# SHI-Labs/SH-GAN

Hardware: AMD Instinct MI355X
Metric: generator images/sec (higher is better)
Workload: dtype f32

## Files before the change

### include/shgan_hip.h

```cpp
#ifndef SHGAN_HIP_H
#define SHGAN_HIP_H
#include <stddef.h>
#include <stdint.h>
#ifdef __cplusplus
extern "C" {
#endif

#define SHG_OK 0
#define SHG_ERR_ARG (-1)
#define SHG_ERR_LAUNCH (-2)
#define SHG_ERR_UNSUPPORTED (-3)

int shg_abi_version(void);
const char* shg_last_error(void);
int shg_device_info(int dev, char* buf, int buflen);

int shg_upfirdn2d_out_size(int H, int W, int fh, int fw, int upx, int upy, int downx, int downy, int padx0, int padx1,
                           int pady0, int pady1, int* OH, int* OW);
int shg_upfirdn2d_f32(const float* x, const float* f, float* y, int N, int C, int H, int W, int fh, int fw, int upx, int upy,
                      int downx, int downy, int padx0, int padx1, int pady0, int pady1, int flip, float gain, void* stream);
int shg_upfirdn2d_strided(const void* x, const float* f, void* y, int dtype, int N, int C, int H, int W, const long* x_strides,
                          const long* y_strides, int fh, int fw, long f_stride_y, long f_stride_x, int upx, int upy, int downx, int downy,
                          int padx0, int padx1, int pady0, int pady1, int flip, float gain, void* stream);
int shg_upfirdn2d_epilogue_f32(const float* x, const float* f, float* y, int N, int C, int H, int W, int fh, int fw, int upx,
                               int upy, int downx, int downy, int padx0, int padx1, int pady0, int pady1, int flip, float gain,
                               const float* scale, const float* bias, const float* noise, int noise_mode, float noise_strength,
                               int act, float alpha, float act_gain, float clamp, const float* residual, void* stream);

int shg_bias_act_f32(const float* x, float* y, const float* scale, const float* bias, const float* noise, int noise_mode,
                     float noise_strength, const float* residual, int N, int C, int HW, int act, float alpha, float gain,
                     float clamp, void* stream);
int shg_bias_act_backward_f32(const float* g, const float* y, float* dx, long total, int act, float alpha, float gain, float clamp,
                              void* stream);
int shg_fma_f32(const float* a, const float* b, const float* c, float* y, long total, void* stream);
int shg_fma_bcast(const void* a, const void* b, const void* c, void* y, int nd, const long* shape, const long* sa, const long* sb,
                  const long* sc, int f64, void* stream);
int shg_mul_reduce(const void* g, const void* b, void* out, int nd, int nk, const long* shape, const long* sg, const long* sb,
                   int inner_kept, int f64, void* stream);
int shg_scale_channels_f32(const float* x, const float* s, float* y, int NC, int HW, void* stream);
int shg_sum_partials_f32(const float* part, float* out, int N, int B, int K, void* stream);
int shg_scale_cast_f32_f16(const void* src, void* dst, long n, float gain, int to_half, void* stream);
int shg_planes_to_image_f32(const float* mid, const float* bias, float* y, int N, int C, int H, int W, int lo, int OH, int OW,
                            void* stream);

int shg_conv_weight_prep_f32(const float* w, float* wt, float* wscale, float* wsq, int O, int I, int KH, int KW, int OP,
                             int demod, float gain, int flip, void* stream);
int shg_conv2d_f32(const float* x, const float* wt, float* y, int NB, int I, int O, int OP, int H, int W, int kh, int kw,
                   int mode, int pad, int wgroups, long wstride, const float* in_scale, const float* out_scale,
                   const float* bias, const float* noise, int noise_mode, float noise_strength, int act, float alpha, float gain,
                   float clamp, const float* residual, int out_mode, void* workspace, size_t ws_bytes, void* stream);
size_t shg_conv2d_workspace_bytes(int NB, int I, int O, int H, int W, int kh, int kw, int mode, int pad, int wgroups);
int shg_conv_wino_chunk(void);
int shg_conv_weight_prep_wino_f32(const float* w, const float* wscale, float* wu, int O, int I, int OP, int flip, void* stream);
int shg_conv2d_wino_f32(const float* x, const float* wu, float* y, int NB, int I, int O, int OP, int H, int W,
                        const float* in_scale, const float* out_scale, const float* bias, const float* noise, int noise_mode,
                        float noise_strength, int act, float alpha, float gain, float clamp, const float* residual, void* stream);
size_t shg_conv2d_wino_workspace_bytes(int NB, int I, int O, int OP, int H, int W);
int shg_conv2d_wino_ws_f32(const float* x, const float* wu, float* y, int NB, int I, int O, int OP, int H, int W,
                           const float* in_scale, const float* out_scale, const float* bias, const float* noise, int noise_mode,
                           float noise_strength, int act, float alpha, float gain, float clamp, const float* residual, void* workspace,
                           size_t ws_bytes, void* stream);
long shg_conv_wino4_weight_elems(int OP, int I);
int shg_conv_weight_prep_wino4_f32(const float* w, const float* wscale, float* wu, int O, int I, int OP, int flip, void* stream);
int shg_conv2d_wino4_supported(int NB, int I, int O, int H, int W);
int shg_conv2d_wino4_f32(const float* x, const float* wu, float* y, int NB, int I, int O, int OP, int H, int W,
                         const float* in_scale, const float* out_scale, const float* bias, const float* noise, int noise_mode,
                         float noise_strength, int act, float alpha, float gain, float clamp, const float* residual, void* stream);
size_t shg_conv2d_wino4_workspace_bytes(int NB, int I, int O, int OP, int H, int W);
int shg_conv2d_wino4_ws_f32(const float* x, const float* wu, float* y, int NB, int I, int O, int OP, int H, int W,
                            const float* in_scale, const float* out_scale, const float* bias, const float* noise, int noise_mode,
                            float noise_strength, int act, float alpha, float gain, float clamp, const float* residual, void* workspace,
                            size_t ws_bytes, void* stream);
int shg_conv2d_wino4_route_f32(const float* x, const float* wu, float* y, int NB, int I, int O, int OP, int H, int W,
                               const float* in_scale, const float* out_scale, const float* bias, const float* noise, int noise_mode,
                               float noise_strength, int act, float alpha, float gain, float clamp, const float* residual, int route,
                               void* workspace, size_t ws_bytes, void* stream);
int shg_upfir_planar_f32(const float* mid, const float* f, float* y, int N, int C, int H, int W, int flip, float gain,
                         const float* scale, const float* bias, const float* noise, int noise_mode, float noise_strength,
                         int act, float alpha, float act_gain, float clamp, const float* residual, void* stream);
int shg_upfir_planar_sep_supported(int H, int W);
int shg_upfir_planar_sep_f32(const float* mid, const float* taps_host, float* y, int N, int C, int H, int W, int flip, float gain,
                             const float* scale, const float* bias, const float* noise, int noise_mode, float noise_strength,
                             int act, float alpha, float act_gain, float clamp, const float* residual, void* stream);
int shg_conv_weight_prep_up_poly_f32(const float* w, const float* wscale, float* wu_a, float* wu_b, int O, int I, int OP, int flip,
                                     void* stream);
int shg_conv2d_up_poly_supported(int NB, int I, int O, int H, int W);
int shg_conv2d_up_poly_f32(const float* x, const float* wt, const float* wu_a, const float* wu_b, float* y, int NB, int I, int O,
                           int OP, int H, int W, const float* in_scale, void* stream);
size_t shg_conv2d_up_poly_workspace_bytes(int NB, int I, int O, int OP, int H, int W);
int shg_conv2d_up_poly_ws_f32(const float* x, const float* wt, const float* wu_a, const float* wu_b, float* y, int NB, int I, int O,
                              int OP, int H, int W, const float* in_scale, void* workspace, size_t ws_bytes, void* stream);
int shg_fir_down_planar_f32(const float* x, const float* f, float* y, int N, int C, int H, int W, int PP, int flip, float gain,
                            void* stream);
int shg_fir_pad2_sep_supported(int H, int W, int PP);
int shg_fir_pad2_sep_f32(const float* x, const float* taps_host, float* y, int N, int C, int H, int W, int PP, int flip, float gain,
                         void* stream);
int shg_fir_resample2_sep_supported(int H, int W, int up);
int shg_fir_resample2_sep_f32(const float* x, const float* taps_host, float* y, int N, int C, int H, int W, int up, int flip, float gain,
                              void* stream);
int shg_conv_weight_prep_down_poly_f32(const float* w, const float* wscale, float* wu_a, float* wu_b, int O, int I, int OP, int flip,
                                       void* stream);
int shg_conv2d_down_poly_supported(int NB, int I, int O, int OH, int OW);
int shg_conv2d_down_poly_f32(const float* xp, const float* wu_a, const float* wu_b, float* y, int NB, int I, int O, int OP, int OH,
                             int OW, int PP, const float* in_scale, const float* bias, int act, float alpha, float gain,
                             float clamp, const float* residual, void* stream);
int shg_conv1x1_thin_in_f32(const float* x, const float* w, const float* bias, float* y, int N, int I, int O, int HW, float wgain,
                            int act, float alpha, float gain, float clamp, void* stream);
int shg_torgb_f32(const float* x, const float* w, const float* styles, const float* bias, const float* base_up, const float* f,
                  float* y, int N, int I, int O, int H, int W, void* stream);

int shg_dense_f32(const float* x, const float* w, const float* b, float* y, int N, int K, int O, int ldx, int ldy, float wgain,
                  float bgain, int act, float alpha, float gain, float clamp, void* stream);
int shg_matmul_nn_f32(const float* a, const float* b, float* out, int N, int M, int K, int lda, int ldo, float scale, void* stream);
int shg_matmul_tn_f32(const float* a, const float* b, float* out, float* colsum, int N, int M, int K, int lda, int ldb, float scale,
                      float csum_scale, void* stream);
int shg_demod_weight_f32(const float* w, float* wn, float* wsq, float* sfac, int O, int I, int K, int prenorm, void* stream);
int shg_demod_weight_backward_f32(const float* wn, const float* sfac, const float* gwn, const float* gwsq, float* gw, int O, int I, int K,
                                  void* stream);
int shg_style_factors_f32(const float* s, const float* wsq, float* sn, float* d, float* aux, int N, int I, int O, int prenorm, void* stream);
int shg_style_factors_backward_f32(const float* sn, const float* d, const float* wsq, const float* aux, const float* gsn, const float* gd,
                                   float* gs, float* gwsq, float* partq, int N, int I, int O, int prenorm, void* stream);
int shg_normalize_2nd_moment_f32(const float* x, float* y, int N, int K, float eps, void* stream);
int shg_modconv_style_prep_f32(const float* styles, int ld, const float* wsq, float* s_out, float* dcoef, int N, int I, int O,
                               int OP, int demod, float pre_gain, void* stream);

typedef struct {
    const float* x1; const float* x2; const float* w; const float* b; float* y;
    int ld1, ld2, K1, K2, O, ldy;
    float wgain, bgain;
} shg_dense_group;
int shg_dense_grouped_f32(const shg_dense_group* groups, int G, int N, void* stream);
typedef struct {
    const float* styles; const float* wsq; float* s_out; float* dcoef;
    int ld, I, O, OP, demod;
    float pre_gain;
} shg_style_group;
int shg_modconv_style_prep_grouped_f32(const shg_style_group* groups, int G, int N, void* stream);

int shg_shu_rfft2_shift_f32(const float* x, long x_batch_stride, float* T, int N, int C, void* stream);
size_t shg_conv2d_wgrad_workspace_bytes(int NB, int I, int O, int OH, int OW, int kh, int kw);
int shg_conv2d_wgrad_f32(const float* x, const float* g, float* dw, int NB, int I, int O, int H, int W, int OH, int OW,
                         int kh, int kw, int stride, int pad, void* workspace, size_t ws_bytes, void* stream);
int shg_conv2d_wgrad_wino_supported(int H, int W, int OH, int OW, int kh, int kw, int stride, int pad);
size_t shg_conv2d_wgrad_wino_workspace_bytes(int NB, int I, int O, int H, int W);
int shg_conv2d_wgrad_wino_f32(const float* x, const float* g, float* dw, int NB, int I, int O, int H, int W, void* workspace,
                              size_t ws_bytes, void* stream);
int shg_shu_spectral_f32(const float* T, const float* w0p, const float* b0, const float* w1p, const float* cw, float* S,
                         int N, int C2, int P, int bands, void* stream);
int shg_shu_split_irfft2_f32(const float* Y, const float* cw, const float* const* gauss, float* const* out,
                             const long* out_batch_stride, int N, int C, int bands, int accumulate, void* stream);
int shg_shu_split_adjoint_f32(const float* const* g, const long* g_batch_stride, const float* const* gauss, float* GS, int N, int C,
                              void* stream);
int shg_shu_rfft2_shift_n_f32(const float* x, long x_batch_stride, float* T, int N, int C, int size, void* stream);
int shg_shu_spectral_n_f32(const float* T, const float* w0p, const float* b0, const float* w1p, const float* cw, float* S,
                           int N, int C2, int P, int bands, void* stream);
int shg_shu_split_irfft2_n_f32(const float* Y, const float* cw, const float* const* gauss, float* const* out,
                               const long* out_batch_stride, int N, int C, int bands, int accumulate, int size, const int* res,
                               int levels, void* stream);
int shg_shu_split_adjoint_n_f32(const float* const* g, const long* g_batch_stride, const float* const* gauss, float* GS, int N, int C,
                                int size, const int* res, int levels, void* stream);

int shg_composite_u8(const float* x4, const float* img, uint8_t* out, int N, int H, int W, void* stream);

int shg_assemble_input_f32(const float* real, const float* mask, float* x, int N, int H, int W, void* stream);
int shg_assemble_input_u8(const uint8_t* real, const float* mask, const float* lut, float* x, int N, int H, int W, void* stream);

int shg_mask_raster_f32(const int* records, const int* offsets, const int* flips, const int* disc_table, int max_half, float* mask,
                        int* holes, int B, int s, void* stream);
int shg_mask_raster_box_f32(const int* records, const int* offsets, const int* flips, const int* disc_table, int max_half, const int* boxes,
                            float* mask, int* holes, int B, int s, void* stream);

int shg_mask_lama_f32(const int* records_host, const int* offsets_host, const int* records, const int* offsets, const int* circle_table,
                      int rmax, float* mask, int* holes, int B, int total, int s, void* stream);

// ... 104 lines not shown
```

### sh-gan_amd/_lib.py

```python
import ctypes
import os

import torch

_HERE = os.path.dirname(os.path.abspath(__file__))
LIB_PATH = os.path.join(_HERE, 'lib', 'libshgan_hip.so')
ABI_VERSION = 40

c_fp = ctypes.c_void_p
c_i = ctypes.c_int
c_f = ctypes.c_float
c_l = ctypes.c_long
c_pp = ctypes.POINTER(ctypes.c_void_p)



class DenseGroup(ctypes.Structure):
    _fields_ = [('x1', c_fp), ('x2', c_fp), ('w', c_fp), ('b', c_fp), ('y', c_fp),
                ('ld1', c_i), ('ld2', c_i), ('K1', c_i), ('K2', c_i), ('O', c_i), ('ldy', c_i),
                ('wgain', c_f), ('bgain', c_f)]


class StyleGroup(ctypes.Structure):
    _fields_ = [('styles', c_fp), ('wsq', c_fp), ('s_out', c_fp), ('dcoef', c_fp),
                ('ld', c_i), ('I', c_i), ('O', c_i), ('OP', c_i), ('demod', c_i), ('pre_gain', c_f)]


class IncConv(ctypes.Structure):
    _fields_ = [('x', c_fp), ('w', c_fp), ('bias', c_fp), ('y', c_fp)] + [
        (n, c_i) for n in ('I', 'H', 'W', 'x_ctot', 'x_coff', 'O', 'kh', 'kw', 'sh', 'sw', 'ph', 'pw', 'OH', 'OW', 'y_ctot', 'y_coff', 'splitk')]


_SIGS = {
    'shg_abi_version': [],
    'shg_device_info': [c_i, ctypes.c_char_p, c_i],
    'shg_upfirdn2d_out_size': [c_i] * 12 + [ctypes.POINTER(c_i), ctypes.POINTER(c_i)],
    'shg_upfirdn2d_f32': [c_fp, c_fp, c_fp] + [c_i] * 15 + [c_f, c_fp],
    'shg_upfirdn2d_strided': [c_fp, c_fp, c_fp, c_i, c_i, c_i, c_i, c_i, ctypes.POINTER(c_l), ctypes.POINTER(c_l), c_i, c_i, c_l, c_l] + [c_i] * 9
                             + [c_f, c_fp],
    'shg_upfirdn2d_epilogue_f32': [c_fp, c_fp, c_fp] + [c_i] * 15 + [c_f, c_fp, c_fp, c_fp, c_i, c_f, c_i, c_f, c_f, c_f, c_fp, c_fp],
    'shg_bias_act_f32': [c_fp, c_fp, c_fp, c_fp, c_fp, c_i, c_f, c_fp, c_i, c_i, c_i, c_i, c_f, c_f, c_f, c_fp],
    'shg_fma_f32': [c_fp, c_fp, c_fp, c_fp, c_l, c_fp],
    'shg_fma_bcast': [c_fp, c_fp, c_fp, c_fp, c_i] + [ctypes.POINTER(c_l)] * 4 + [c_i, c_fp],
    'shg_mul_reduce': [c_fp, c_fp, c_fp, c_i, c_i] + [ctypes.POINTER(c_l)] * 3 + [c_i, c_i, c_fp],
    'shg_scale_channels_f32': [c_fp, c_fp, c_fp, c_i, c_i, c_fp],
    'shg_sum_partials_f32': [c_fp, c_fp, c_i, c_i, c_i, c_fp],
    'shg_scale_cast_f32_f16': [c_fp, c_fp, c_l, c_f, c_i, c_fp],
    'shg_planes_to_image_f32': [c_fp, c_fp, c_fp, c_i, c_i, c_i, c_i, c_i, c_i, c_i, c_fp],
    'shg_conv_weight_prep_f32': [c_fp, c_fp, c_fp, c_fp, c_i, c_i, c_i, c_i, c_i, c_i, c_f, c_i, c_fp],
    'shg_conv2d_f32': [c_fp, c_fp, c_fp] + [c_i] * 11 + [c_l, c_fp, c_fp, c_fp, c_fp, c_i, c_f, c_i, c_f, c_f, c_f, c_fp, c_i,
                       c_fp, ctypes.c_size_t, c_fp],
    'shg_conv2d_workspace_bytes': [c_i] * 10,
    'shg_conv_wino_chunk': [],
    'shg_conv_weight_prep_wino_f32': [c_fp, c_fp, c_fp, c_i, c_i, c_i, c_i, c_fp],
    'shg_conv2d_wino_f32': [c_fp, c_fp, c_fp] + [c_i] * 6 + [c_fp, c_fp, c_fp, c_fp, c_i, c_f, c_i, c_f, c_f, c_f, c_fp, c_fp],
    'shg_conv2d_wino_ws_f32': [c_fp, c_fp, c_fp] + [c_i] * 6 + [c_fp, c_fp, c_fp, c_fp, c_i, c_f, c_i, c_f, c_f, c_f, c_fp, c_fp, ctypes.c_size_t, c_fp],
    'shg_conv2d_wino_workspace_bytes': [c_i] * 6,
    'shg_conv_wino4_weight_elems': [c_i, c_i],
    'shg_conv_weight_prep_wino4_f32': [c_fp, c_fp, c_fp, c_i, c_i, c_i, c_i, c_fp],
    'shg_conv2d_wino4_supported': [c_i] * 5,
    'shg_conv2d_wino4_f32': [c_fp, c_fp, c_fp] + [c_i] * 6 + [c_fp, c_fp, c_fp, c_fp, c_i, c_f, c_i, c_f, c_f, c_f, c_fp, c_fp],
    'shg_conv2d_wino4_ws_f32': [c_fp, c_fp, c_fp] + [c_i] * 6 + [c_fp, c_fp, c_fp, c_fp, c_i, c_f, c_i, c_f, c_f, c_f, c_fp, c_fp, ctypes.c_size_t, c_fp],
    'shg_conv2d_wino4_route_f32': [c_fp, c_fp, c_fp] + [c_i] * 6 + [c_fp, c_fp, c_fp, c_fp, c_i, c_f, c_i, c_f, c_f, c_f, c_fp, c_i, c_fp, ctypes.c_size_t, c_fp],
    'shg_conv2d_wino4_workspace_bytes': [c_i] * 6,
    'shg_upfir_planar_f32': [c_fp, c_fp, c_fp, c_i, c_i, c_i, c_i, c_i, c_f, c_fp, c_fp, c_fp, c_i, c_f, c_i, c_f, c_f, c_f, c_fp, c_fp],
    'shg_upfir_planar_sep_supported': [c_i, c_i],
    'shg_upfir_planar_sep_f32': [c_fp, ctypes.POINTER(c_f), c_fp, c_i, c_i, c_i, c_i, c_i, c_f, c_fp, c_fp, c_fp, c_i, c_f, c_i, c_f, c_f, c_f, c_fp, c_fp],
    'shg_conv1x1_thin_in_f32': [c_fp, c_fp, c_fp, c_fp, c_i, c_i, c_i, c_i, c_f, c_i, c_f, c_f, c_f, c_fp],
    'shg_torgb_f32': [c_fp, c_fp, c_fp, c_fp, c_fp, c_fp, c_fp, c_i, c_i, c_i, c_i, c_i, c_fp],
    'shg_dense_f32': [c_fp, c_fp, c_fp, c_fp, c_i, c_i, c_i, c_i, c_i, c_f, c_f, c_i, c_f, c_f, c_f, c_fp],
    'shg_demod_weight_f32': [c_fp, c_fp, c_fp, c_fp, c_i, c_i, c_i, c_i, c_fp],
    'shg_demod_weight_backward_f32': [c_fp, c_fp, c_fp, c_fp, c_fp, c_i, c_i, c_i, c_fp],
    'shg_style_factors_f32': [c_fp, c_fp, c_fp, c_fp, c_fp, c_i, c_i, c_i, c_i, c_fp],
    'shg_style_factors_backward_f32': [c_fp, c_fp, c_fp, c_fp, c_fp, c_fp, c_fp, c_fp, c_fp, c_i, c_i, c_i, c_i, c_fp],
    'shg_matmul_nn_f32': [c_fp, c_fp, c_fp, c_i, c_i, c_i, c_i, c_i, c_f, c_fp],
    'shg_matmul_tn_f32': [c_fp, c_fp, c_fp, c_fp, c_i, c_i, c_i, c_i, c_i, c_f, c_f, c_fp],
    'shg_normalize_2nd_moment_f32': [c_fp, c_fp, c_i, c_i, c_f, c_fp],
    'shg_modconv_style_prep_f32': [c_fp, c_i, c_fp, c_fp, c_fp, c_i, c_i, c_i, c_i, c_i, c_f, c_fp],
    'shg_dense_grouped_f32': [ctypes.POINTER(DenseGroup), c_i, c_i, c_fp],
    'shg_modconv_style_prep_grouped_f32': [ctypes.POINTER(StyleGroup), c_i, c_i, c_fp],
    'shg_shu_rfft2_shift_f32': [c_fp, c_l, c_fp, c_i, c_i, c_fp],
    'shg_bias_act_backward_f32': [c_fp, c_fp, c_fp, c_l, c_i, c_f, c_f, c_f, c_fp],
    'shg_conv2d_wgrad_workspace_bytes': [c_i] * 7,
    'shg_conv2d_wgrad_f32': [c_fp, c_fp, c_fp] + [c_i] * 11 + [c_fp, ctypes.c_size_t, c_fp],
    'shg_conv2d_wgrad_wino_supported': [c_i] * 8,
    'shg_conv2d_wgrad_wino_workspace_bytes': [c_i] * 5,
    'shg_conv2d_wgrad_wino_f32': [c_fp, c_fp, c_fp] + [c_i] * 5 + [c_fp, ctypes.c_size_t, c_fp],
    'shg_shu_spectral_f32': [c_fp] * 6 + [c_i] * 4 + [c_fp],
    'shg_shu_split_irfft2_f32': [c_fp, c_fp, c_pp, c_pp, ctypes.POINTER(c_l), c_i, c_i, c_i, c_i, c_fp],
    'shg_shu_split_adjoint_f32': [c_pp, ctypes.POINTER(c_l), c_pp, c_fp, c_i, c_i, c_fp],
    'shg_shu_rfft2_shift_n_f32': [c_fp, c_l, c_fp, c_i, c_i, c_i, c_fp],
    'shg_shu_spectral_n_f32': [c_fp] * 6 + [c_i] * 4 + [c_fp],
    'shg_shu_split_irfft2_n_f32': [c_fp, c_fp, c_pp, c_pp, ctypes.POINTER(c_l), c_i, c_i, c_i, c_i, c_i, ctypes.POINTER(c_i), c_i, c_fp],
    'shg_shu_split_adjoint_n_f32': [c_pp, ctypes.POINTER(c_l), c_pp, c_fp, c_i, c_i, c_i, ctypes.POINTER(c_i), c_i, c_fp],
    'shg_composite_u8': [c_fp, c_fp, c_fp, c_i, c_i, c_i, c_fp],
    'shg_assemble_input_f32': [c_fp, c_fp, c_fp, c_i, c_i, c_i, c_fp],
    'shg_assemble_input_u8': [c_fp, c_fp, c_fp, c_fp, c_i, c_i, c_i, c_fp],
    'shg_conv_weight_prep_up_poly_f32': [c_fp, c_fp, c_fp, c_fp, c_i, c_i, c_i, c_i, c_fp],
    'shg_conv2d_up_poly_supported': [c_i, c_i, c_i, c_i, c_i],
    'shg_conv2d_up_poly_f32': [c_fp, c_fp, c_fp, c_fp, c_fp, c_i, c_i, c_i, c_i, c_i, c_i, c_fp, c_fp],
    'shg_conv2d_up_poly_ws_f32': [c_fp, c_fp, c_fp, c_fp, c_fp] + [c_i] * 6 + [c_fp, c_fp, ctypes.c_size_t, c_fp],
    'shg_conv2d_up_poly_workspace_bytes': [c_i] * 6,
    'shg_fir_down_planar_f32': [c_fp, c_fp, c_fp, c_i, c_i, c_i, c_i, c_i, c_i, c_f, c_fp],
    'shg_fir_pad2_sep_supported': [c_i, c_i, c_i],
    'shg_fir_resample2_sep_supported': [c_i, c_i, c_i],
    'shg_fir_resample2_sep_f32': [c_fp, ctypes.POINTER(c_f), c_fp, c_i, c_i, c_i, c_i, c_i, c_i, c_f, c_fp],
    'shg_fir_pad2_sep_f32': [c_fp, ctypes.POINTER(c_f), c_fp, c_i, c_i, c_i, c_i, c_i, c_i, c_f, c_fp],
    'shg_conv_weight_prep_down_poly_f32': [c_fp, c_fp, c_fp, c_fp, c_i, c_i, c_i, c_i, c_fp],
    'shg_conv2d_down_poly_supported': [c_i, c_i, c_i, c_i, c_i],
    'shg_conv2d_down_poly_f32': [c_fp, c_fp, c_fp, c_fp, c_i, c_i, c_i, c_i, c_i, c_i, c_i, c_fp, c_fp, c_i, c_f, c_f, c_f, c_fp, c_fp],
    'shg_mask_raster_f32': [c_fp, c_fp, c_fp, c_fp, c_i, c_fp, c_fp, c_i, c_i, c_fp],
    'shg_mask_raster_box_f32': [c_fp, c_fp, c_fp, c_fp, c_i, c_fp, c_fp, c_fp, c_i, c_i, c_fp],
    'shg_mask_lama_f32': [c_fp, c_fp, c_fp, c_fp, c_fp, c_i, c_fp, c_fp, c_i, c_i, c_i, c_fp],
    'shg_fid_accumulate_f64': [c_fp, c_i, c_fp, c_fp, c_i, c_i, c_i, c_fp],
    'shg_inception_frontend_f32': [c_fp, c_fp, c_f, c_f, c_fp, c_i, c_i, c_i, c_fp],
    'shg_inception_packed_weight_elems': [c_i] * 4,
    'shg_inception_weight_prep_f32': [c_fp, c_fp, c_fp, c_fp, c_i, c_i, c_i, c_i, c_fp],
    'shg_inception_conv_workspace_bytes': [ctypes.POINTER(IncConv), c_i, c_i],
    'shg_inception_conv_f32': [ctypes.POINTER(IncConv), c_i, c_i, c_fp, ctypes.c_size_t, c_fp],
    'shg_inception_pool_f32': [c_fp, c_fp] + [c_i] * 9 + [c_fp],
    'shg_inception_mean_f32': [c_fp, c_fp, c_i, c_i, c_i, c_fp],
    'shg_inception_head_f32': [c_fp, c_fp, c_fp, c_fp, c_i, c_i, c_i, c_fp],
    'shg_kid_workspace_bytes': [c_i, c_i],
    'shg_kid_sums_f64': [c_fp, c_fp, c_i, c_i, c_i, c_i, c_fp, c_fp, c_i, c_i, c_fp, ctypes.c_size_t, c_fp, c_fp],
    'shg_is_accumulate_f64': [c_fp, c_fp, c_fp, c_i, c_i, c_i, c_fp],
    'shg_pr_workspace_bytes': [c_i, c_i, c_i],
    'shg_pr_radii_f16': [c_fp, c_i, c_i, c_i, c_fp, ctypes.c_size_t, c_fp, c_fp],
    'shg_pr_inside_f16': [c_fp, c_i, c_fp, c_i, c_i, c_fp, c_fp, ctypes.c_size_t, c_fp, c_fp],
    'shg_vgg16_frontend_f32': [c_fp, c_fp, c_f, c_f, ctypes.POINTER(c_f), ctypes.POINTER(c_f), c_fp, c_i, c_i, c_i, c_fp],
    'shg_vgg16_maxpool2_f32': [c_fp, c_fp, c_i, c_i, c_i, c_i, c_fp],
    'shg_lpips_conv1_weight_prep_f32': [c_fp, c_fp, c_fp, c_fp, c_fp],
    'shg_lpips_conv1_f32': [c_fp, c_fp, c_f, c_f, ctypes.POINTER(c_f), ctypes.POINTER(c_f), c_fp, c_fp, c_fp, c_i, c_i, c_i, c_fp],
    'shg_lpips_head_scratch_bytes': [c_i] * 3,
    'shg_lpips_head_f32': [c_fp, c_fp, c_fp, c_i, c_i, c_i, c_i, c_fp, ctypes.c_size_t, c_fp, c_fp],
    'shg_lpips_scaling_f32': [c_fp, c_fp, c_f, c_f, ctypes.POINTER(c_f), ctypes.POINTER(c_f), c_fp, c_i, c_i, c_i, c_fp],
    'shg_ppl_frontend_f32': [c_fp, c_fp, c_i, c_i, c_i, c_i, c_i, c_i, ctypes.POINTER(c_f), ctypes.POINTER(c_f), c_fp],
    'shg_adam_tick': [c_fp, c_i, c_fp, c_i, c_fp, c_fp, c_fp],
    'shg_adam_buckets_f32': [c_fp, c_i, c_l, c_fp, c_f, c_i, c_i, c_fp],
    'shg_ema_lerp_f32': [c_fp, c_i, c_l, c_fp, c_fp],
    'shg_image_metrics_scratch_bytes': [c_i] * 4,
    'shg_image_metrics': [c_fp, c_fp, c_f, c_f, c_fp, c_fp, c_f, c_f] + [c_i] * 6 + [c_fp, ctypes.c_size_t, c_fp, c_fp, c_fp],
    'shg_resize_bicubic_u8': [c_fp, c_l, c_fp, c_l, c_fp, c_i, c_i, c_i, c_i, c_i, c_fp],
    'shg_resize_fit_pad_u8': [c_fp, c_l, c_fp, c_l, c_fp, c_i, c_i, c_i, c_i, c_i, c_fp],
    'shg_randcrop_bicubic_ragged_f32': [c_fp, c_l, ctypes.POINTER(c_i), c_fp, c_fp, c_fp, c_i, c_i, c_fp],
    'shg_randcrop_bicubic_planar_f32': [c_fp, c_l, ctypes.POINTER(c_i), c_fp, c_fp, c_fp, c_i, c_i, c_fp],
    'shg_minibatch_std_f32': [c_fp, c_fp, c_fp, c_i, c_i, c_i, c_i, c_i, c_i, c_fp],
    'shg_conv2d_f16': [c_fp, c_fp, c_fp, c_fp] + [c_i] * 12 + [c_fp],
    'shg_conv2d_f16_needs_clear': [c_i] * 5,
    'shg_conv2d_f16_fused': [c_fp, c_fp, c_fp] + [c_i] * 12 + [c_fp, c_fp, c_fp, c_i, c_f, c_fp, c_i, c_f, c_f, c_f, c_fp, c_fp],
    'shg_conv2d_f16_packed_weight_elems': [c_i] * 3,
    'shg_conv2d_f16_pack_weight': [c_fp, c_fp, c_i, c_i, c_i, c_fp],
    'shg_conv2d_f16_pack_weight_oihw': [c_fp, c_fp, c_i, c_i, c_i, c_i, c_i, c_fp],
    'shg_conv2d_f16_set_routes': [c_i],
    'shg_conv2d_wgrad_f16_workspace_bytes': [c_i] * 6,
    'shg_conv2d_wgrad_f16': [c_fp, c_fp, c_fp] + [c_i] * 10 + [c_fp, ctypes.c_size_t, c_fp],
    'shg_upfirdn2d_f16': [c_fp, c_fp, c_fp] + [c_i] * 15 + [c_f, c_fp],
    'shg_relayout_f32_f16': [c_fp, c_fp, c_i, c_i, c_l, c_i, c_fp],
    'shg_bias_act_f16': [c_fp, c_fp, c_fp, c_l, c_i, c_i, c_f, c_f, c_f, c_fp],
    'shg_bias_act_backward_f16': [c_fp, c_fp, c_fp, c_l, c_i, c_f, c_f, c_f, c_fp],
    'shg_modtail_backward_f32_blocks': [c_l],
    'shg_modtail_backward_f32_cslices': [c_i, c_i, c_l],
    'shg_modtail_backward_f32': [c_fp] * 9 + [c_i, c_i, c_l, c_i, c_f, c_f, c_f, c_fp],
    'shg_modtail_f16': [c_fp, c_fp, c_fp, c_i, c_fp, c_fp, c_i, c_l, c_i, c_i, c_f, c_f, c_f, c_fp],
    'shg_modtail_backward_f16_blocks': [c_l, c_i],
    'shg_modtail_backward_f16': [c_fp] * 9 + [c_i, c_l, c_i, c_i, c_f, c_f, c_f, c_fp],
}

_lib = None


class ShgError(RuntimeError):
    """Raised when a C-ABI call returns a negative status (mirrors TORCH_CHECK -> RuntimeError)."""


def get_lib():
    global _lib
    if _lib is not None:
        return _lib
    if not os.path.exists(LIB_PATH):
        raise RuntimeError(
            f'{LIB_PATH} not found: the HIP extension is not built. Run `python sh-gan_amd/build.py` '
            '(or __graft_entry__.build()). There is deliberately no CPU / PyTorch fallback.')
    lib = ctypes.CDLL(LIB_PATH)
    for name, args in _SIGS.items():
        fn = getattr(lib, name)
        fn.argtypes = args
        fn.restype = c_i
    lib.shg_last_error.argtypes = []
    lib.shg_last_error.restype = ctypes.c_char_p
    lib.shg_conv2d_workspace_bytes.restype = ctypes.c_size_t
    lib.shg_conv2d_wgrad_workspace_bytes.restype = ctypes.c_size_t
    lib.shg_conv2d_wino_workspace_bytes.restype = ctypes.c_size_t
    lib.shg_conv2d_wino4_workspace_bytes.restype = ctypes.c_size_t
    lib.shg_conv2d_up_poly_workspace_bytes.restype = ctypes.c_size_t
    lib.shg_conv2d_wgrad_wino_workspace_bytes.restype = ctypes.c_size_t
    lib.shg_conv2d_wgrad_f16_workspace_bytes.restype = ctypes.c_size_t
    lib.shg_image_metrics_scratch_bytes.restype = ctypes.c_size_t
    lib.shg_lpips_head_scratch_bytes.restype = ctypes.c_size_t
    lib.shg_inception_conv_workspace_bytes.restype = ctypes.c_size_t
    lib.shg_kid_workspace_bytes.restype = ctypes.c_size_t
    lib.shg_pr_workspace_bytes.restype = ctypes.c_size_t
    lib.shg_inception_packed_weight_elems.restype = c_l
    lib.shg_conv2d_f16_packed_weight_elems.restype = c_l
    lib.shg_conv_wino4_weight_elems.restype = c_l
    ver = lib.shg_abi_version()
    if ver != ABI_VERSION:
        raise RuntimeError(f'libshgan_hip.so ABI {ver} != expected {ABI_VERSION}: rebuild with sh-gan_amd/build.py')
    _lib = lib
    return lib


def exported_symbols():
    return sorted(list(_SIGS.keys()) + ['shg_last_error'])


def check(rc, what=''):
    if rc != 0:
        msg = get_lib().shg_last_error().decode(errors='replace')
        raise ShgError(f'{what}: {msg} (code {rc})')
```

### sh-gan_amd/csrc/conv_wino_poly.hip

```cpp
#include "wino_common.h"
#include <stdlib.h>
#include <type_traits>

__device__ __attribute__((aligned(16))) float shg_poly_zeros[64];

struct PolySub {
    const float* wu;
    int nby, nbx;
    int tiles_x, tiles_y;
    int n_ttiles;
};
struct PolyParams {
    const float* x;
    float* y;
    const float* in_scale;
    int NB, I, O, OP, H, W;
    int n_otiles, nchunk;
    PolySub a, b;
    const float* wt;
    int IPK, n_strip_tiles;
    int PH2, PP;
    const float* bias;
    const float* residual;
    int act;
    float alpha, gain, clamp;
    int cps;
    long part_stride;
};

namespace poly {
constexpr int KC = 8, BO = 64, BT = 64;
constexpr int V_SZ = 16 * KC * BT;
constexpr int NT = 1024;
constexpr int NXF = KC;

enum { UA = 0, UB = 1, DA = 2, DB = 3 };

template <int SCHEME, int TY, int TX, int NBX>
struct Geo {
    static constexpr bool A = SCHEME == UA || SCHEME == DA;
    static_assert(NBX > 0 || TY * TX == BT, "64 blocks per tile");
    static_assert(NBX == 0 || A, "flat tiling is for the 3x3 blocks of schemes UA / DA");
    static constexpr int BS = A ? 3 : 2;
    static constexpr int RMAX = NBX ? (NBX - 1 + BT + NBX - 1) / NBX : TY;
    static constexpr int PH = A ? 3 * RMAX + 1 : 2 * TY + 1;
    static constexpr int PW = SCHEME == UA ? ((3 * (NBX ? NBX : TX) + 1 + 3 + 3) / 4) * 4
                            : SCHEME == DA ? (NBX ? ((3 * NBX + 1 + 3) / 4) * 4 : ((3 * TX + 1 + 3 + 3) / 4) * 4)
                            : 2 * TX + 4;
    static constexpr int DB_W0 = 2 * TX, DB_W1 = 2 * TX + 4, DB_W2 = 2 * TX;
    static constexpr int DB_N0 = (2 * TY + 1) * DB_W0, DB_N1 = 2 * TY * DB_W1, DB_N2 = 2 * TY * DB_W2;
    static constexpr int RP = SCHEME == DB ? DB_N0 + DB_N1 + DB_N2 : PH * PW;
    static constexpr int PW4 = PW / 4, PATCH4 = RP / 4, R_SZ = KC * RP;
    static constexpr int NPIECE = (PATCH4 + 63) / 64;
};
}

template <int SCHEME, int TY, int TX, int NBX>
__device__ __forceinline__ void poly_body(const PolyParams& p, const PolySub& q, const int bid, float* __restrict__ Vl,
                                          float* __restrict__ Rl) {
    using namespace poly;
    using G = Geo<SCHEME, TY, TX, NBX>;
    constexpr int PW = G::PW, PW4 = G::PW4, PATCH4 = G::PATCH4, RP = G::RP, R_SZ = G::R_SZ, BS = G::BS, NPIECE = G::NPIECE;
    constexpr bool FLAT = NBX > 0;
    constexpr bool DOWN = SCHEME == DA || SCHEME == DB;
    const int c0 = DOWN ? 0 : blockIdx.y * p.cps, nch = DOWN ? p.nchunk : min(p.cps, p.nchunk - c0), iend = min(p.I, (c0 + nch) * poly::KC);

    const int tid = threadIdx.x;
    const int lane = tid & 63, wave = __builtin_amdgcn_readfirstlane(tid >> 6);
    const int l31 = lane & 31, half = lane >> 5;

    const int nwork = q.n_ttiles * p.n_otiles;
    const int work = shg_xcd_remap(bid, nwork);
    const int otile = work / q.n_ttiles;
    const int ttile = work - otile * q.n_ttiles;
    const int txb = ttile % q.tiles_x;
    const int tyb = (ttile / q.tiles_x) % q.tiles_y;
    const int n = ttile / (q.tiles_x * q.tiles_y);
    const int id0 = txb * BT;
    const int by0 = FLAT ? id0 / (NBX ? NBX : 1) : tyb * TY, bx0 = FLAT ? 0 : txb * TX;
    const int o0 = otile * BO;
    const int HW = DOWN ? p.PH2 * p.PP : p.H * p.W;
    const int wy0 = DOWN ? BS * by0 : BS * by0 - 1;
    const int wx0 = SCHEME == UA ? ((3 * bx0 - 1) & ~3) : SCHEME == DA ? ((3 * bx0) & ~3) : SCHEME == UB ? 2 * bx0 - 4 : 2 * bx0;
    const int coff = (DOWN ? BS * bx0 : BS * bx0 - 1) - wx0;

    const bool xformer = wave < NXF;
    constexpr int NLD = 16 - NXF;
    constexpr int CPL = (KC + NLD - 1) / NLD;
    int roff[NPIECE];
#pragma unroll
    for (int j = 0; j < NPIECE; ++j) {
        const int e = j * 64 + lane;
        if constexpr (SCHEME == DB) {
            constexpr int N0 = G::DB_N0 / 4, N1 = G::DB_N1 / 4, W0 = G::DB_W0 / 4, W1 = G::DB_W1 / 4, W2 = G::DB_W2 / 4;
            const int pl = e < N0 ? 1 : (e < N0 + N1 ? 2 : 3);
            const int r4 = e < N0 ? e : (e < N0 + N1 ? e - N0 : e - N0 - N1);
            const int w4 = pl == 1 ? W0 : (pl == 2 ? W1 : W2);
            const int py = r4 / w4, p4 = r4 - py * w4;
            const int iy = wy0 + py, ix = wx0 + 4 * p4;
            const bool ok = e < PATCH4 && iy < p.PH2 && ix + 3 < p.PP;
            roff[j] = ok ? (pl * p.NB + n) * p.I * HW + iy * p.PP + ix : -1;
        } else {
            const int py = e / PW4, p4 = e - py * PW4;
            const int iy = wy0 + py, ix = wx0 + 4 * p4;
            if constexpr (SCHEME == DA) {
                const bool ok = e < PATCH4 && iy < p.PH2 && ix + 3 < p.PP;
                roff[j] = ok ? n * p.I * HW + iy * p.PP + ix : -1;
            } else {
                const bool ok = e < PATCH4 && iy >= 0 && iy < p.H && ix >= 0 && ix + 3 < p.W;
                roff[j] = ok ? n * p.I * HW + iy * p.W + ix : -1;
// ... 89 lines not shown
            for (int cc = 1; cc < 3; ++cc) {
                vb[(0 * 2 + cc - 1) * KC * BT] = d[0][cc] - d[1][cc];
                vb[(1 * 2 + cc - 1) * KC * BT] = d[1][cc];
                vb[(2 * 2 + cc - 1) * KC * BT] = d[2][cc] - d[1][cc];
            }
#pragma unroll
            for (int r = 1; r < 3; ++r) {
                vb[(6 + (r - 1) * 3 + 0) * KC * BT] = d[r][0] - d[r][1];
                vb[(6 + (r - 1) * 3 + 1) * KC * BT] = d[r][1];
                vb[(6 + (r - 1) * 3 + 2) * KC * BT] = d[r][2] - d[r][1];
            }
#pragma unroll
            for (int r = 1; r < 3; ++r)
#pragma unroll
                for (int cc = 1; cc < 3; ++cc) vb[(12 + (r - 1) * 2 + cc - 1) * KC * BT] = d[r][cc];
        }
    };

    f32x16 acc[2][2];
#pragma unroll
    for (int ob = 0; ob < 2; ++ob)
#pragma unroll
        for (int tb = 0; tb < 2; ++tb)
#pragma unroll
            for (int r = 0; r < 16; ++r) acc[ob][tb][r] = 0.f;
    const float* bbase = Vl + (wave * KC + half) * BT + l31;

    load_u(ua, 0);
    if (!xformer) {
        dma_raw(0, 0);
        if (nch > 1) dma_raw(1, 1);
    }
    asm volatile("s_waitcnt vmcnt(0)" ::: "memory");
    __syncthreads();
    if (xformer) transform(0, 0);
    __syncthreads();

    float b[2][2], apend[2];
    auto mma = [&](float a0, float a1, int buf) __attribute__((always_inline)) {
#pragma unroll
        for (int tb = 0; tb < 2; ++tb) acc[0][tb] = __builtin_amdgcn_mfma_f32_32x32x2f32(a0, b[buf][tb], acc[0][tb], 0, 0, 0);
#pragma unroll
        for (int tb = 0; tb < 2; ++tb) acc[1][tb] = __builtin_amdgcn_mfma_f32_32x32x2f32(a1, b[buf][tb], acc[1][tb], 0, 0, 0);
    };
    auto chunk = [&](auto par, int c) __attribute__((always_inline)) {
        constexpr int PAR = decltype(par)::value;
        f32x4 (&ucur)[NU] = PAR ? ub : ua;
        f32x4 (&unxt)[NU] = PAR ? ua : ub;
        const bool more = c + 1 < nch;
        const float* bb = bbase + PAR * V_SZ;
        auto fetch = [&](int ks, int buf) __attribute__((always_inline)) {
#pragma unroll
            for (int tb = 0; tb < 2; ++tb) b[buf][tb] = bb[(ks * 2) * BT + tb * 32];
        };
        fetch(0, 0);
        __builtin_amdgcn_sched_barrier(0);
        if (c > 0) mma(apend[0], apend[1], 1);
        __builtin_amdgcn_sched_barrier(0);
        if (more) load_u(unxt, c + 1);
        if (!xformer) {
            if (c + 2 < nch) dma_raw(c + 2, PAR);
        } else if (more) {
            transform(c + 1, PAR ^ 1);
        }
        __builtin_amdgcn_sched_barrier(0);
#pragma unroll
        for (int ks = 0; ks < KC / 2 - 1; ++ks) {
            fetch(ks + 1, (ks + 1) & 1);
            __builtin_amdgcn_sched_barrier(0);
            mma(ucur[(ks * 2) / 4][(ks * 2) % 4], ucur[(ks * 2 + 1) / 4][(ks * 2 + 1) % 4], ks & 1);
        }
        apend[0] = ucur[(KC - 2) / 4][(KC - 2) % 4];
        apend[1] = ucur[(KC - 1) / 4][(KC - 1) % 4];
        asm volatile("s_waitcnt lgkmcnt(0)" ::: "memory");
        __syncthreads();
    };
    for (int c = 0; c < nch; c += 2) {
        chunk(std::integral_constant<int, 0>{}, c);
        if (c + 1 < nch) chunk(std::integral_constant<int, 1>{}, c + 1);
    }
    mma(apend[0], apend[1], 1);

    float* Mx = Vl;
    const int PWg = DOWN ? p.W : p.W + 1;
    const long plane = DOWN ? (long)p.H * p.W : (long)(p.H + 1) * PWg;
    const int o_l = tid >> 5, t_l = tid & 31;
    f32x2 pre_part[SCHEME == DB ? 4 : 1][2], pre_res[SCHEME == DB ? 4 : 1][2];
    float pre_bias[2] = {0.f, 0.f};
    const ShgAct actc = shg_act_make(p.act, p.alpha, p.gain, p.clamp);
    if constexpr (SCHEME == DB) {
#pragma unroll
        for (int pass = 0; pass < 4; ++pass) {
            const int ob = pass >> 1, t = (pass & 1) * 32 + t_l;
            const int by = by0 + t / TX, bx = bx0 + t % TX;
            const int o = min(o0 + ob * 32 + o_l, p.O - 1);
            if ((pass & 1) == 0) pre_bias[ob] = p.bias ? p.bias[o] : 0.f;
#pragma unroll
            for (int j = 0; j < 2; ++j) {
                pre_part[pass][j] = f32x2{0.f, 0.f};
                pre_res[pass][j] = f32x2{0.f, 0.f};
                if (by < q.nby && bx < q.nbx && 2 * by + j < p.H) {
                    const long off = ((long)n * p.O + o) * plane + (long)(2 * by + j) * PWg + 2 * bx;
                    pre_part[pass][j] = *reinterpret_cast<const f32x2*>(p.y + off);
                    if (p.residual) pre_res[pass][j] = *reinterpret_cast<const f32x2*>(p.residual + off);
                }
            }
        }
    }
#pragma unroll
    for (int pass = 0; pass < 4; ++pass) {
        const int ob = pass >> 1, tb = pass & 1;
#pragma unroll
        for (int r = 0; r < 16; ++r) {
            const int row = (r & 3) + 8 * (r >> 2) + 4 * half;
            Mx[(wave * 32 + row) * 32 + l31] = acc[ob][tb][r];
        }
        __syncthreads();
        float m[16];
#pragma unroll
        for (int xi = 0; xi < 16; ++xi) m[xi] = Mx[(xi * 32 + o_l) * 32 + t_l];
        const int t = tb * 32 + t_l;
        const int by = FLAT ? (id0 + t) / (NBX ? NBX : 1) : by0 + t / TX, bx = FLAT ? (id0 + t) % (NBX ? NBX : 1) : bx0 + t % TX;
        const int o = o0 + ob * 32 + o_l;
        if (o < p.O && by < q.nby && bx < q.nbx) {
            float* yb = p.y + (DOWN ? 0 : blockIdx.y * p.part_stride) + ((long)n * p.O + o) * plane;
            const long pstride = (long)p.NB * p.O * plane;
            if constexpr (G::A) {
                float t3[3][4];
#pragma unroll
                for (int cc = 0; cc < 4; ++cc) {
                    t3[0][cc] = m[0 * 4 + cc] + m[1 * 4 + cc] + m[2 * 4 + cc];
                    t3[1][cc] = m[1 * 4 + cc] - m[2 * 4 + cc];
                    t3[2][cc] = m[1 * 4 + cc] + m[2 * 4 + cc] - m[3 * 4 + cc];
                }
                constexpr int EXT = DOWN ? 0 : 1;
#pragma unroll
                for (int i = 0; i < 3; ++i) {
                    const int u = 3 * by + i;
                    if (u >= p.H + EXT) continue;
                    const float y0 = t3[i][0] + t3[i][1] + t3[i][2], y1 = t3[i][1] - t3[i][2], y2 = t3[i][1] + t3[i][2] - t3[i][3];
                    float* yr = yb + (long)u * PWg + 3 * bx;
                    yr[0] = y0;
                    if (3 * bx + 1 < p.W + EXT) yr[1] = y1;
                    if (3 * bx + 2 < p.W + EXT) yr[2] = y2;
                }
            } else if constexpr (SCHEME == DB) {
                const int p0 = 2 * by, q0 = 2 * bx;
                const float bs = pre_bias[ob];
#pragma unroll
                for (int j = 0; j < 2; ++j) {
                    if (p0 + j >= p.H) continue;
                    float* yr = yb + (long)(p0 + j) * PWg + q0;
                    const f32x2 part = pre_part[pass][j];
                    const f32x2 rs = pre_res[pass][j];
                    f32x2 out;
#pragma unroll
                    for (int cc = 0; cc < 2; ++cc) {
                        float v = part[cc] + m[j * 2 + cc] + m[(j + 1) * 2 + cc]
                                + m[6 + j * 3 + cc] + m[6 + j * 3 + cc + 1]
                                + m[12 + j * 2 + cc] + bs;
                        out[cc] = shg_act_apply(v, actc) + rs[cc];
                    }
                    *reinterpret_cast<f32x2*>(yr) = out;
                }
            } else {
                const int u0 = 2 * by, v0 = 2 * bx;
                float* yeo = yb + pstride + (long)u0 * PWg + v0;
                float* yoe = yb + 2 * pstride + (long)u0 * PWg + v0;
                float* yoo = yb + 3 * pstride + (long)u0 * PWg + v0;
#pragma unroll
                for (int cc = 0; cc < 2; ++cc) {
                    yeo[cc] = m[0 * 2 + cc] + m[1 * 2 + cc];
                    yeo[PWg + cc] = m[1 * 2 + cc] + m[2 * 2 + cc];
                }
#pragma unroll
                for (int r = 0; r < 2; ++r) {
                    yoe[r * PWg] = m[6 + r * 3] + m[6 + r * 3 + 1];
                    yoe[r * PWg + 1] = m[6 + r * 3 + 1] + m[6 + r * 3 + 2];
                    yoo[r * PWg] = m[12 + r * 2];
                    yoo[r * PWg + 1] = m[12 + r * 2 + 1];
                }
            }
        }
        if (pass < 3) __syncthreads();
    }
}

__device__ __forceinline__ void poly_strip_body(const PolyParams& p, const int tile, const int wave, float* __restrict__ redbuf) {
    float (*red)[16][64] = reinterpret_cast<float (*)[16][64]>(redbuf);
    const float* wt = p.wt;
    const int IPK = p.IPK;
    const int lane = threadIdx.x & 63;
    const int l31 = lane & 31, half = lane >> 5;
    const int nseg_r = (p.W + 31) / 32, nseg_c = (p.H + 31) / 32;
    const int no32 = p.OP / 32;
    const bool live = tile < p.n_strip_tiles;
    int seg = tile % (nseg_r + nseg_c);
    const int ot32 = (tile / (nseg_r + nseg_c)) % no32;
    const int n = live ? tile / ((nseg_r + nseg_c) * no32) : 0;
    const bool col = seg >= nseg_r;
    if (col) seg -= nseg_r;
    const int len = col ? p.H : p.W;
    const int pos = seg * 32 + l31;
    const int tap = col ? 1 * 3 + 2 : 2 * 3 + 1;
    const int HW = p.H * p.W;
    const bool pok = live && pos < len;
    const float* xb = p.x + (long)n * p.I * HW + (pok ? (col ? pos * p.W + p.W - 1 : (p.H - 1) * p.W + pos) : 0);
    const float* wb = wt + ((long)(ot32 >> 1) * IPK + tap) * 64 + (ot32 & 1) * 32 + l31;
    const float* sb = p.in_scale ? p.in_scale + (long)n * p.I : nullptr;
    const int i_lo = blockIdx.y * p.cps * poly::KC, i_hi = min(p.I, i_lo + p.cps * poly::KC);
    const int kper = ((i_hi - i_lo + 7) / 8) * 2;
    const int kbeg = i_lo + wave * kper, kend = min(i_hi, kbeg + kper);
    f32x16 acc;
#pragma unroll
    for (int r = 0; r < 16; ++r) acc[r] = 0.f;
    for (int i0 = kbeg; i0 < kend; i0 += 32) {
        float a[16], bv[16];
#pragma unroll
        for (int k = 0; k < 16; ++k) {
            const int ic = i0 + 2 * k + half;
            const int i = min(ic, p.I - 1);
            a[k] = wb[(long)i * 9 * 64];
            bv[k] = xb[(long)i * HW];
            if (sb) bv[k] *= sb[i];
            if (ic >= kend) a[k] = 0.f;
            if (ic >= kend || !pok) bv[k] = 0.f;
        }
#pragma unroll
        for (int k = 0; k < 16; ++k) acc = __builtin_amdgcn_mfma_f32_32x32x2f32(a[k], bv[k], acc, 0, 0, 0);
    }
#pragma unroll
    for (int r = 0; r < 16; ++r) red[wave][r][lane] = acc[r];
    __syncthreads();
    if (!pok) return;
    const int PWg = p.W + 1;
    const long plane = (long)(p.H + 1) * PWg;
    const long pix = col ? (long)pos * PWg + p.W : (long)p.H * PWg + pos;
    float* yb = p.y + blockIdx.y * p.part_stride + (long)(col ? 2 : 1) * p.NB * p.O * plane + (long)n * p.O * plane + pix;
#pragma unroll
    for (int rr = 0; rr < 4; ++rr) {
        const int r = wave * 4 + rr;
        const float v = red[0][r][lane] + red[1][r][lane] + red[2][r][lane] + red[3][r][lane];
        const int o = ot32 * 32 + (r & 3) + 8 * (r >> 2) + 4 * half;
        if (o < p.O) yb[(long)o * plane] = v;
    }
}

template <int ATY, int ATX, int ANBX, int BTY, int BTX>
__global__ __launch_bounds__(1024) void conv_poly_up_kernel(const PolyParams p) {
    using namespace poly;
    using GA = Geo<UA, ATY, ATX, ANBX>;
    using GB = Geo<UB, BTY, BTX, 0>;
    constexpr int R_MAX = GA::R_SZ > GB::R_SZ ? GA::R_SZ : GB::R_SZ;
    __shared__ __attribute__((aligned(16))) float Vl[2 * V_SZ];
    __shared__ __attribute__((aligned(16))) float Rl[2 * R_MAX];
    const int nA = p.a.n_ttiles * p.n_otiles, nB = p.b.n_ttiles * p.n_otiles;
    if ((int)blockIdx.x < nA) poly_body<UA, ATY, ATX, ANBX>(p, p.a, blockIdx.x, Vl, Rl);
    else if ((int)blockIdx.x < nA + nB) poly_body<UB, BTY, BTX, 0>(p, p.b, blockIdx.x - nA, Vl, Rl);
    else {
        const int wave = threadIdx.x >> 6;
        poly_strip_body(p, (blockIdx.x - nA - nB) * 4 + (wave >> 2), wave & 3, Vl + (wave >> 2) * 4 * 16 * 64);
    }
}

template <int SCHEME, int TY, int TX, int NBX>
__global__ __launch_bounds__(1024) void conv_poly_down_kernel(const PolyParams p) {
    using namespace poly;
    using G = Geo<SCHEME, TY, TX, NBX>;
    __shared__ __attribute__((aligned(16))) float Vl[2 * V_SZ];
    __shared__ __attribute__((aligned(16))) float Rl[2 * G::R_SZ];
    poly_body<SCHEME, TY, TX, NBX>(p, SCHEME == DA ? p.a : p.b, blockIdx.x, Vl, Rl);
}

__global__ __launch_bounds__(256) void poly_weight_kernel(const float* w, const float* scale, float* wu, int O, int I, int OP,
                                                          int nchunk, int flip, int scheme) {
    constexpr int KC = poly::KC;
    const long e = (long)blockIdx.x * 256 + threadIdx.x;
    const long total = (long)OP * nchunk * KC;
    if (e >= total) return;
    const int o = (int)(e % OP);
    const int i = (int)(e / OP);
    float g[3][3];
#pragma unroll
    for (int t = 0; t < 9; ++t) {
        const int tt = flip ? 8 - t : t;
        g[t / 3][t % 3] = (o < O && i < I) ? w[((long)o * I + i) * 9 + tt] * scale[o] : 0.f;
    }
    float u[16];
    if (scheme == poly::UA) {
        const float q00 = g[2][2], q01 = g[2][0], q10 = g[0][2], q11 = g[0][0];
        float gq[4][2];
        gq[0][0] = q00; gq[0][1] = q01;
        gq[1][0] = 0.5f * (q00 + q10); gq[1][1] = 0.5f * (q01 + q11);
        gq[2][0] = 0.5f * (q00 - q10); gq[2][1] = 0.5f * (q01 - q11);
        gq[3][0] = q10; gq[3][1] = q11;
#pragma unroll
        for (int r = 0; r < 4; ++r) {
            u[r * 4 + 0] = gq[r][0];
            u[r * 4 + 1] = 0.5f * (gq[r][0] + gq[r][1]);
            u[r * 4 + 2] = 0.5f * (gq[r][0] - gq[r][1]);
            u[r * 4 + 3] = gq[r][1];
        }
    } else if (scheme == poly::UB) {
        const float g0 = g[0][1], g1 = g[2][1];
        const float h0 = g[1][0], h1 = g[1][2];
#pragma unroll
        for (int cc = 0; cc < 2; ++cc) { u[0 * 2 + cc] = g1; u[1 * 2 + cc] = g0 + g1; u[2 * 2 + cc] = g0; }
#pragma unroll
        for (int r = 0; r < 2; ++r) { u[6 + r * 3 + 0] = h1; u[6 + r * 3 + 1] = h0 + h1; u[6 + r * 3 + 2] = h0; }
#pragma unroll
        for (int k = 0; k < 4; ++k) u[12 + k] = g[1][1];
    } else if (scheme == poly::DA) {
        const float q00 = g[0][0], q01 = g[0][2], q10 = g[2][0], q11 = g[2][2];
        float gq[4][2];
        gq[0][0] = q00; gq[0][1] = q01;
        gq[1][0] = 0.5f * (q00 + q10); gq[1][1] = 0.5f * (q01 + q11);
        gq[2][0] = 0.5f * (q00 - q10); gq[2][1] = 0.5f * (q01 - q11);
        gq[3][0] = q10; gq[3][1] = q11;
#pragma unroll
        for (int r = 0; r < 4; ++r) {
            u[r * 4 + 0] = gq[r][0];
            u[r * 4 + 1] = 0.5f * (gq[r][0] + gq[r][1]);
            u[r * 4 + 2] = 0.5f * (gq[r][0] - gq[r][1]);
            u[r * 4 + 3] = gq[r][1];
        }
    } else {
        const float g0 = g[0][1], g1 = g[2][1];
        const float h0 = g[1][0], h1 = g[1][2];
#pragma unroll
        for (int cc = 0; cc < 2; ++cc) { u[0 * 2 + cc] = g0; u[1 * 2 + cc] = g0 + g1; u[2 * 2 + cc] = g1; }
#pragma unroll
        for (int r = 0; r < 2; ++r) { u[6 + r * 3 + 0] = h0; u[6 + r * 3 + 1] = h0 + h1; u[6 + r * 3 + 2] = h1; }
#pragma unroll
        for (int k = 0; k < 4; ++k) u[12 + k] = g[1][1];
    }
    const int k = i % KC, chunk = i / KC;
    const int ln = (k & 1) * 32 + (o & 31), slot = (k >> 1) * 2 + ((o & 63) >> 5);
    float* dst = wu + ((((long)(o >> 6) * nchunk + chunk) * 16) * 64 + ln) * KC + slot;
#pragma unroll
    for (int xi = 0; xi < 16; ++xi) dst[(long)xi * 64 * KC] = u[xi];
}

extern "C" int shg_conv_weight_prep_up_poly_f32(const float* w, const float* wscale, float* wu_a, float* wu_b, int O, int I, int OP,
                                                int flip, void* stream) {
    SHG_CHECK_ARG(w && wscale && wu_a && wu_b, "weight_prep_up_poly: null pointer");
    SHG_CHECK_ARG(O >= 1 && I >= 1 && OP % 64 == 0 && OP >= O, "weight_prep_up_poly: bad shape");
    const int nchunk = shg_cdiv(I, poly::KC);
    const long total = (long)OP * nchunk * poly::KC;
    hipLaunchKernelGGL(poly_weight_kernel, dim3(shg_cdiv(total, 256)), dim3(256), 0, (hipStream_t)stream, w, wscale, wu_a, O, I, OP,
                       nchunk, flip, (int)poly::UA);
    SHG_CHECK_LAUNCH();
    hipLaunchKernelGGL(poly_weight_kernel, dim3(shg_cdiv(total, 256)), dim3(256), 0, (hipStream_t)stream, w, wscale, wu_b, O, I, OP,
                       nchunk, flip, (int)poly::UB);
    SHG_CHECK_LAUNCH();
    return SHG_OK;
}

extern "C" int shg_conv2d_up_poly_supported(int NB, int I, int O, int H, int W) {
    return (H >= 16 && W >= 16 && H % 2 == 0 && W % 4 == 0 && I <= 128 * poly::KC && NB >= 1 && O >= 1) ? 1 : 0;
}

static int up_poly_plan(PolyParams& p, int NB, int I, int OP, int H, int W) {
    p.n_otiles = OP / 64; p.nchunk = shg_cdiv(I, poly::KC);
    const bool bwide = W >= 32;
    p.b.nby = H / 2; p.b.nbx = W / 2;
    p.b.tiles_x = shg_cdiv(p.b.nbx, bwide ? 16 : 8); p.b.tiles_y = shg_cdiv(p.b.nby, bwide ? 4 : 8);
    p.b.n_ttiles = p.b.tiles_x * p.b.tiles_y * NB;
    p.a.nby = shg_cdiv(H + 1, 3); p.a.nbx = shg_cdiv(W + 1, 3);
    const bool flat = bwide && (p.a.nbx == 11 || p.a.nbx == 22 || p.a.nbx == 43);
    const long w88 = (long)shg_cdiv(p.a.nbx, 8) * shg_cdiv(p.a.nby, 8), w416 = (long)shg_cdiv(p.a.nbx, 16) * shg_cdiv(p.a.nby, 4);
    const bool wide = bwide && w416 < w88;
    if (flat) { p.a.tiles_x = shg_cdiv(p.a.nby * p.a.nbx, 64); p.a.tiles_y = 1; }
    else { p.a.tiles_x = shg_cdiv(p.a.nbx, wide ? 16 : 8); p.a.tiles_y = shg_cdiv(p.a.nby, wide ? 4 : 8); }
    p.a.n_ttiles = p.a.tiles_x * p.a.tiles_y * NB;
    p.IPK = (I + 31) / 32 * 32 * 9;
    p.n_strip_tiles = (shg_cdiv(W, 32) + shg_cdiv(H, 32)) * (OP / 32) * NB;
    if (!bwide) return 0;
    if (flat) return p.a.nbx == 11 ? 1 : (p.a.nbx == 22 ? 2 : 3);
    return wide ? 4 : 5;
}

extern "C" size_t shg_conv2d_up_poly_workspace_bytes(int NB, int I, int O, int OP, int H, int W) {
    if (!shg_conv2d_up_poly_supported(NB, I, O, H, W) || OP < 64) return 0;
    PolyParams p{};
    up_poly_plan(p, NB, I, OP, H, W);
    return shg_wino_split_bytes((long)(p.a.n_ttiles + p.b.n_ttiles) * p.n_otiles, p.nchunk, (size_t)4 * NB * O * (H + 1) * (W + 1) * sizeof(float));
}

extern "C" int shg_conv2d_up_poly_ws_f32(const float* x, const float* wt, const float* wu_a, const float* wu_b, float* y, int NB, int I,
                                         int O, int OP, int H, int W, const float* in_scale, void* workspace, size_t ws_bytes, void* stream) {
    SHG_CHECK_ARG(x && wt && wu_a && wu_b && y, "conv2d_up_poly: null pointer");
    SHG_CHECK_ARG(shg_conv2d_up_poly_supported(NB, I, O, H, W), "conv2d_up_poly: unsupported geometry (use shg_conv2d_f32 mode 2)");
    SHG_CHECK_ARG(OP % 64 == 0 && OP >= O, "conv2d_up_poly: OP must be a multiple of 64 and >= O");
    SHG_CHECK_ARG((long)NB * I * H * W < 2147483647L && 4L * NB * O * (H + 1) * (W + 1) < 2147483647L, "conv2d_up_poly: tensor too large");
    SHG_CHECK_ARG((reinterpret_cast<uintptr_t>(x) & 15) == 0, "conv2d_up_poly: x must be 16-byte aligned");
    hipStream_t s = (hipStream_t)stream;
    PolyParams p{};
    p.x = x; p.y = y; p.in_scale = in_scale;
    p.NB = NB; p.I = I; p.O = O; p.OP = OP; p.H = H; p.W = W;
    p.a.wu = wu_a; p.b.wu = wu_b; p.wt = wt;
    const int variant = up_poly_plan(p, NB, I, OP, H, W);
    const int ks = shg_wino_split((long)(p.a.n_ttiles + p.b.n_ttiles) * p.n_otiles, p.nchunk, (size_t)4 * NB * O * (H + 1) * (W + 1) * sizeof(float),
                                  workspace, ws_bytes, shg_addr(workspace) | shg_addr(y), &p.y, &p.cps, &p.part_stride);
    const dim3 grid((p.a.n_ttiles + p.b.n_ttiles) * p.n_otiles + shg_cdiv(p.n_strip_tiles, 4), ks);
    if (variant == 0) hipLaunchKernelGGL((conv_poly_up_kernel<8, 8, 0, 8, 8>), grid, dim3(poly::NT), 0, s, p);
    else if (variant == 1) hipLaunchKernelGGL((conv_poly_up_kernel<1, 64, 11, 4, 16>), grid, dim3(poly::NT), 0, s, p);
    else if (variant == 2) hipLaunchKernelGGL((conv_poly_up_kernel<1, 64, 22, 4, 16>), grid, dim3(poly::NT), 0, s, p);
    else if (variant == 3) hipLaunchKernelGGL((conv_poly_up_kernel<1, 64, 43, 4, 16>), grid, dim3(poly::NT), 0, s, p);
    else if (variant == 4) hipLaunchKernelGGL((conv_poly_up_kernel<4, 16, 0, 4, 16>), grid, dim3(poly::NT), 0, s, p);
    else hipLaunchKernelGGL((conv_poly_up_kernel<8, 8, 0, 4, 16>), grid, dim3(poly::NT), 0, s, p);
    SHG_CHECK_LAUNCH();
    if (ks > 1) {
        shg_launch_wino_split_reduce((const float*)workspace, y, ks, 4 * NB, O, H + 1, W + 1, nullptr, nullptr, nullptr, 0, 0.f, 0, 0.f, 1.f, -1.f, nullptr, s);
        SHG_CHECK_LAUNCH();
    }
    return SHG_OK;
}

extern "C" int shg_conv2d_up_poly_f32(const float* x, const float* wt, const float* wu_a, const float* wu_b, float* y, int NB, int I,
                                      int O, int OP, int H, int W, const float* in_scale, void* stream) {
    return shg_conv2d_up_poly_ws_f32(x, wt, wu_a, wu_b, y, NB, I, O, OP, H, W, in_scale, nullptr, 0, stream);
}


extern "C" int shg_conv_weight_prep_down_poly_f32(const float* w, const float* wscale, float* wu_a, float* wu_b, int O, int I, int OP,
                                                  int flip, void* stream) {
    SHG_CHECK_ARG(w && wscale && wu_a && wu_b, "weight_prep_down_poly: null pointer");
    SHG_CHECK_ARG(O >= 1 && I >= 1 && OP % 64 == 0 && OP >= O, "weight_prep_down_poly: bad shape");
    const int nchunk = shg_cdiv(I, poly::KC);
    const long total = (long)OP * nchunk * poly::KC;
    hipLaunchKernelGGL(poly_weight_kernel, dim3(shg_cdiv(total, 256)), dim3(256), 0, (hipStream_t)stream, w, wscale, wu_a, O, I, OP,
                       nchunk, flip, (int)poly::DA);
    SHG_CHECK_LAUNCH();
    hipLaunchKernelGGL(poly_weight_kernel, dim3(shg_cdiv(total, 256)), dim3(256), 0, (hipStream_t)stream, w, wscale, wu_b, O, I, OP,
                       nchunk, flip, (int)poly::DB);
    SHG_CHECK_LAUNCH();
    return SHG_OK;
}

extern "C" int shg_conv2d_down_poly_supported(int NB, int I, int O, int OH, int OW) {
    return (OH >= 16 && OW >= 16 && OW % 4 == 0 && OH % 2 == 0 && I <= 128 * poly::KC && NB >= 1 && O >= 1) ? 1 : 0;
}

extern "C" int shg_conv2d_down_poly_f32(const float* xp, const float* wu_a, const float* wu_b, float* y, int NB, int I, int O, int OP,
                                        int OH, int OW, int PP, const float* in_scale, const float* bias, int act, float alpha,
                                        float gain, float clamp, const float* residual, void* stream) {
    SHG_CHECK_ARG(xp && wu_a && wu_b && y, "conv2d_down_poly: null pointer");
    SHG_CHECK_ARG(shg_conv2d_down_poly_supported(NB, I, O, OH, OW), "conv2d_down_poly: unsupported geometry (use shg_conv2d_f32 mode 1)");
    SHG_CHECK_ARG(OP % 64 == 0 && OP >= O, "conv2d_down_poly: OP must be a multiple of 64 and >= O");
    SHG_CHECK_ARG(PP % 4 == 0 && PP >= OW + 1, "conv2d_down_poly: plane pitch must be a multiple of 4 and >= OW + 1");
    SHG_CHECK_ARG(4L * NB * I * (OH + 1) * PP < 2147483647L && (long)NB * O * OH * OW < 2147483647L, "conv2d_down_poly: tensor too large");
    SHG_CHECK_ARG(((reinterpret_cast<uintptr_t>(xp) & 15) | (reinterpret_cast<uintptr_t>(y) & 7) | (reinterpret_cast<uintptr_t>(residual) & 7)) == 0,
                  "conv2d_down_poly: xp must be 16-byte, y / residual 8-byte aligned");
    hipStream_t s = (hipStream_t)stream;
    PolyParams p{};
    p.x = xp; p.y = y; p.in_scale = in_scale; p.bias = bias; p.residual = residual;
    p.NB = NB; p.I = I; p.O = O; p.OP = OP; p.H = OH; p.W = OW; p.PH2 = OH + 1; p.PP = PP;
    p.act = act; p.alpha = alpha; p.gain = gain; p.clamp = clamp;
    p.n_otiles = OP / 64; p.nchunk = shg_cdiv(I, poly::KC);
    p.cps = p.nchunk; p.part_stride = 0;
    p.a.wu = wu_a; p.a.nby = shg_cdiv(OH, 3); p.a.nbx = shg_cdiv(OW, 3);
    const bool flat = p.a.nbx == 11 || p.a.nbx == 22 || p.a.nbx == 43;
    const long w88 = (long)shg_cdiv(p.a.nbx, 8) * shg_cdiv(p.a.nby, 8), w416 = (long)shg_cdiv(p.a.nbx, 16) * shg_cdiv(p.a.nby, 4);
    const bool wide = OW >= 32 && w416 < w88;
    if (flat) { p.a.tiles_x = shg_cdiv(p.a.nby * p.a.nbx, 64); p.a.tiles_y = 1; }
    else { p.a.tiles_x = shg_cdiv(p.a.nbx, wide ? 16 : 8); p.a.tiles_y = shg_cdiv(p.a.nby, wide ? 4 : 8); }
    p.a.n_ttiles = p.a.tiles_x * p.a.tiles_y * NB;
    const dim3 ga(p.a.n_ttiles * p.n_otiles);
    if (flat && p.a.nbx == 11) hipLaunchKernelGGL((conv_poly_down_kernel<poly::DA, 1, 64, 11>), ga, dim3(poly::NT), 0, s, p);
    else if (flat && p.a.nbx == 22) hipLaunchKernelGGL((conv_poly_down_kernel<poly::DA, 1, 64, 22>), ga, dim3(poly::NT), 0, s, p);
    else if (flat) hipLaunchKernelGGL((conv_poly_down_kernel<poly::DA, 1, 64, 43>), ga, dim3(poly::NT), 0, s, p);
    else if (wide) hipLaunchKernelGGL((conv_poly_down_kernel<poly::DA, 4, 16, 0>), ga, dim3(poly::NT), 0, s, p);
    else hipLaunchKernelGGL((conv_poly_down_kernel<poly::DA, 8, 8, 0>), ga, dim3(poly::NT), 0, s, p);
    SHG_CHECK_LAUNCH();
    const bool bwide = OW >= 32, bxwide = OW >= 64;
    p.b.wu = wu_b; p.b.nby = OH / 2; p.b.nbx = OW / 2;
    p.b.tiles_x = shg_cdiv(p.b.nbx, bxwide ? 32 : (bwide ? 16 : 8)); p.b.tiles_y = shg_cdiv(p.b.nby, bxwide ? 2 : (bwide ? 4 : 8));
    p.b.n_ttiles = p.b.tiles_x * p.b.tiles_y * NB;
    const dim3 gb(p.b.n_ttiles * p.n_otiles);
    if (bxwide) hipLaunchKernelGGL((conv_poly_down_kernel<poly::DB, 2, 32, 0>), gb, dim3(poly::NT), 0, s, p);
    else if (bwide) hipLaunchKernelGGL((conv_poly_down_kernel<poly::DB, 4, 16, 0>), gb, dim3(poly::NT), 0, s, p);
    else hipLaunchKernelGGL((conv_poly_down_kernel<poly::DB, 8, 8, 0>), gb, dim3(poly::NT), 0, s, p);
    SHG_CHECK_LAUNCH();
    return SHG_OK;
}
```

### sh-gan_amd/csrc/fir_march.h

```cpp
#pragma once
#include <hip/hip_runtime.h>

struct FirMarchParams {
    const float* x;
    float* y;
    int NC, H, W;
    int mode;
    int pitch, ph2;
    int R, nseg;
    int LPG, G;
    int nitem;
    float a[4], b[4];
};

template <int V> struct FmIC { static constexpr int value = V; };

__device__ __forceinline__ float fm_shr1(float v, float fill) {
    return __builtin_bit_cast(float, __builtin_amdgcn_update_dpp(__builtin_bit_cast(int, fill), __builtin_bit_cast(int, v), 0x138, 0xf, 0xf, false));
}
__device__ __forceinline__ float fm_shl1(float v, float fill) {
    return __builtin_bit_cast(float, __builtin_amdgcn_update_dpp(__builtin_bit_cast(int, fill), __builtin_bit_cast(int, v), 0x130, 0xf, 0xf, false));
}
__device__ __forceinline__ float fm_lane(float v, int l) {
    return __builtin_bit_cast(float, __builtin_amdgcn_readlane(__builtin_bit_cast(int, v), l));
// ... 116 lines not shown
    const float b0 = p.b[0], b1 = p.b[1], b2 = p.b[2], b3 = p.b[3];
    float4 pf[B][K];
    float4 hr[4][K];
    float he[4];
    auto load_row = [&](float4 (&dst)[K], int iy) __attribute__((always_inline)) {
        const int iyc = min(max(iy, 0), p.H - 1);
        const float* src = xb + (long)iyc * p.W;
#pragma unroll
        for (int k = 0; k < K; ++k)
            dst[k] = (DBG & 1) ? make_float4(1.f, 2.f, 3.f, (float)iyc) : *reinterpret_cast<const float4*>(src + 256 * k);
    };
    const long plane_elems = (long)p.ph2 * p.pitch;
    const int w2 = p.W >> 1, npad = p.pitch - w2;
    auto step = [&](auto J, int i) __attribute__((always_inline)) {
        constexpr int jb = decltype(J)::value, j = jb & 3;
        const int iy = r0 - 2 + i;
        const bool rok = iy >= 0 && iy < p.H;
        float4 c[K];
#pragma unroll
        for (int k = 0; k < K; ++k) {
            c[k].x = rok ? pf[jb][k].x : 0.f; c[k].y = rok ? pf[jb][k].y : 0.f;
            c[k].z = rok ? pf[jb][k].z : 0.f; c[k].w = rok ? pf[jb][k].w : 0.f;
        }
#pragma unroll
        for (int k = 0; k < K; ++k) {
            const float fz = k > 0 ? fm_lane(c[k - 1].z, 63) : 0.f, fw = k > 0 ? fm_lane(c[k - 1].w, 63) : 0.f;
            const float fx = k + 1 < K ? fm_lane(c[k + 1].x, 0) : 0.f;
            const float pz = fm_shr1(c[k].z, fz), pw = fm_shr1(c[k].w, fw), nx = fm_shl1(c[k].x, fx);
            hr[j][k].x = a0 * pz + a1 * pw + a2 * c[k].x + a3 * c[k].y;
            hr[j][k].y = a0 * pw + a1 * c[k].x + a2 * c[k].y + a3 * c[k].z;
            hr[j][k].z = a0 * c[k].x + a1 * c[k].y + a2 * c[k].z + a3 * c[k].w;
            hr[j][k].w = a0 * c[k].y + a1 * c[k].z + a2 * c[k].w + a3 * nx;
        }
        he[j] = a0 * fm_lane(c[K - 1].z, 63) + a1 * fm_lane(c[K - 1].w, 63);
        const int oy = r0 + i - 3;
        if (i >= 3 && oy < r1 && (!(DBG & 2) || hr[j][0].x == 12345.f)) {
            constexpr int j0 = (j + 1) & 3, j1 = (j + 2) & 3, j2 = (j + 3) & 3;
            float* pe = p.y + ((long)((oy & 1) * 2) * p.NC + plane) * plane_elems + (long)(oy >> 1) * p.pitch;
            float* po = pe + (long)p.NC * plane_elems;
#pragma unroll
            for (int k = 0; k < K; ++k) {
                float4 o;
                o.x = b0 * hr[j0][k].x + b1 * hr[j1][k].x + b2 * hr[j2][k].x + b3 * hr[j][k].x;
                o.y = b0 * hr[j0][k].y + b1 * hr[j1][k].y + b2 * hr[j2][k].y + b3 * hr[j][k].y;
                o.z = b0 * hr[j0][k].z + b1 * hr[j1][k].z + b2 * hr[j2][k].z + b3 * hr[j][k].z;
                o.w = b0 * hr[j0][k].w + b1 * hr[j1][k].w + b2 * hr[j2][k].w + b3 * hr[j][k].w;
                const int c2 = 2 * (lane + 64 * k);
                *reinterpret_cast<float2*>(pe + c2) = make_float2(o.x, o.z);
                *reinterpret_cast<float2*>(po + c2) = make_float2(o.y, o.w);
            }
            const float oe = b0 * he[j0] + b1 * he[j1] + b2 * he[j2] + b3 * he[j];
            for (int t = lane; t < npad; t += 64) {
                pe[w2 + t] = t == 0 ? oe : 0.f;
                po[w2 + t] = 0.f;
            }
        }
    };
    const int nin = r1 - r0 + 3;
    for (int i = 0; i < nin; i += B) {
#pragma unroll
        for (int j = 0; j < B; ++j) load_row(pf[j], r0 - 2 + i + j);
        step(FmIC<0>{}, i);
        step(FmIC<1>{}, i + 1);
        step(FmIC<2>{}, i + 2);
        step(FmIC<3>{}, i + 3);
        if constexpr (B == 8) {
            step(FmIC<4>{}, i + 4);
            step(FmIC<5>{}, i + 5);
            step(FmIC<6>{}, i + 6);
            step(FmIC<7>{}, i + 7);
        }
    }
    if (seg == p.nseg - 1) {
        float* pz = p.y + ((long)2 * p.NC + plane) * plane_elems + (long)(p.ph2 - 1) * p.pitch;
        for (int q = 0; q < 2; ++q, pz += (long)p.NC * plane_elems)
            for (int c = lane; c < p.pitch; c += 64) pz[c] = 0.f;
    }
}

struct FirUpParams {
    const float* mid; float* y;
    const float* scale; const float* bias; const float* noise; const float* residual;
    int NC, C, H, W;
    int noise_mode;
    float noise_strength;
    int act; float alpha, act_gain, clamp;
    int R, nseg, LPG, G, nitem;
    float a[4], b[4];
};

__device__ __forceinline__ float fm_act(float v, int act, float alpha, float gain, float clamp) {
    if (!act) return v;
    v = (v < 0.f ? v * alpha : v) * gain;
    return clamp >= 0.f ? fminf(fmaxf(v, -clamp), clamp) : v;
}

template <int K, int B>
__global__ __launch_bounds__(256) void fir_up_march_kernel(const FirUpParams p) {
    const int lane = threadIdx.x & 63;
    const int item = blockIdx.x * 4 + (threadIdx.x >> 6);
    if (item >= p.nitem) return;
    const int seg = item % p.nseg, pg = item / p.nseg;
    const int g = lane / p.LPG, li = lane - g * p.LPG;
    const int u0 = seg * p.R, u1 = min(u0 + p.R, p.H);
    const int plane_raw = pg * p.G + g;
    const bool lane_on = plane_raw < p.NC;
    const int plane = lane_on ? plane_raw : 0;
    const bool grp = K == 1 && p.LPG < 64;
    const bool gfirst = grp && li == 0, glast = grp && li == p.LPG - 1;
    const int PW = p.W + 1, OW = 2 * p.W, OH = 2 * p.H;
    const long P = (long)(p.H + 1) * PW;
    const float* mb = p.mid + (long)plane * P + 2 * li;
    const long qs = (long)p.NC * P;
    const int n = plane / p.C, ch = plane - n * p.C;
    const float sc = p.scale ? p.scale[plane] : 1.f, bs = p.bias ? p.bias[ch] : 0.f;
    const float* nzb = p.noise_mode == 0 ? nullptr : (p.noise_mode == 1 ? p.noise : p.noise + (long)n * OH * OW);
    const float* rsb = p.residual ? p.residual + (long)plane * OH * OW : nullptr;
    float* yb = p.y + (long)plane * OH * OW;
    const float a0 = p.a[0], a1 = p.a[1], a2 = p.a[2], a3 = p.a[3];
    const float b0 = p.b[0], b1 = p.b[1], b2 = p.b[2], b3 = p.b[3];

    struct Row { float e0[2][K], e1[2][K], o0[2][K], o1[2][K], ew[2]; float4 nz[2][K], rs[2][K]; };
    Row in[B];
    float4 orA[K], erB[K], orB[K];
#pragma unroll
    for (int k = 0; k < K; ++k) orA[k] = erB[k] = orB[k] = make_float4(0.f, 0.f, 0.f, 0.f);

    auto load_step = [&](Row& d, int r) __attribute__((always_inline)) {
        const int rc = min(max(r, 0), p.H);
        const float* src = mb + (long)rc * PW;
#pragma unroll
        for (int a = 0; a < 2; ++a) {
            const float* se = src + (2 * a) * qs;
            const float* so = se + qs;
#pragma unroll
            for (int k = 0; k < K; ++k) {
                d.e0[a][k] = se[128 * k]; d.e1[a][k] = se[128 * k + 1];
                d.o0[a][k] = so[128 * k]; d.o1[a][k] = so[128 * k + 1];
            }
            d.ew[a] = se[p.W - 2 * li];
        }
        const int yc = min(max(2 * (r - 1), 0), OH - 2);
#pragma unroll
        for (int dy = 0; dy < 2; ++dy)
#pragma unroll
            for (int k = 0; k < K; ++k) {
                const long off = (long)(yc + dy) * OW + 4 * (li + 64 * k);
                d.nz[dy][k] = nzb ? *reinterpret_cast<const float4*>(nzb + off) : make_float4(0.f, 0.f, 0.f, 0.f);
                d.rs[dy][k] = rsb ? *reinterpret_cast<const float4*>(rsb + off) : make_float4(0.f, 0.f, 0.f, 0.f);
            }
    };
    auto hfilt = [&](const Row& d, int a, bool ok, float4 (&h)[K]) __attribute__((always_inline)) {
        float e0[K], e1[K], o0[K], o1[K];
#pragma unroll
        for (int k = 0; k < K; ++k) {
            e0[k] = ok ? d.e0[a][k] : 0.f; e1[k] = ok ? d.e1[a][k] : 0.f;
            o0[k] = ok ? d.o0[a][k] : 0.f; o1[k] = ok ? d.o1[a][k] : 0.f;
        }
        const float ew = ok ? d.ew[a] : 0.f;
#pragma unroll
        for (int k = 0; k < K; ++k) {
            const float fo = k > 0 ? fm_lane(o1[k - 1], 63) : 0.f;
            float om1 = fm_shr1(o1[k], fo);
            float e2 = k + 1 < K ? fm_shl1(e0[k], fm_lane(e0[k + 1], 0)) : fm_shl1(e0[k], ew);
            float o2 = fm_shl1(o0[k], k + 1 < K ? fm_lane(o0[k + 1], 0) : 0.f);
            om1 = gfirst ? 0.f : om1; e2 = glast ? ew : e2; o2 = glast ? 0.f : o2;
            h[k].x = a0 * om1 + a1 * e0[k] + a2 * o0[k] + a3 * e1[k];
            h[k].y = a0 * e0[k] + a1 * o0[k] + a2 * e1[k] + a3 * o1[k];
            h[k].z = a0 * o0[k] + a1 * e1[k] + a2 * o1[k] + a3 * e2;
            h[k].w = a0 * e1[k] + a1 * o1[k] + a2 * e2 + a3 * o2;
        }
    };
    auto finish = [&](float v, float nz, float rs) __attribute__((always_inline)) {
        return fm_act(v * sc + nz * p.noise_strength + bs, p.act, p.alpha, p.act_gain, p.clamp) + rs;
    };
    auto step = [&](const Row& d, int t) __attribute__((always_inline)) {
        const int r = u0 - 1 + t;
        float4 ern[K], orn[K];
        hfilt(d, 0, r >= 0 && r <= p.H, ern);
        hfilt(d, 1, r >= 0 && r <= p.H - 1, orn);
        const int u = r - 1;
        if (t >= 2 && u < u1) {
#pragma unroll
            for (int k = 0; k < K; ++k) {
                float4 y0, y1;
                y0.x = b0 * orA[k].x + b1 * erB[k].x + b2 * orB[k].x + b3 * ern[k].x;
                y0.y = b0 * orA[k].y + b1 * erB[k].y + b2 * orB[k].y + b3 * ern[k].y;
                y0.z = b0 * orA[k].z + b1 * erB[k].z + b2 * orB[k].z + b3 * ern[k].z;
                y0.w = b0 * orA[k].w + b1 * erB[k].w + b2 * orB[k].w + b3 * ern[k].w;
                y1.x = b0 * erB[k].x + b1 * orB[k].x + b2 * ern[k].x + b3 * orn[k].x;
                y1.y = b0 * erB[k].y + b1 * orB[k].y + b2 * ern[k].y + b3 * orn[k].y;
                y1.z = b0 * erB[k].z + b1 * orB[k].z + b2 * ern[k].z + b3 * orn[k].z;
                y1.w = b0 * erB[k].w + b1 * orB[k].w + b2 * ern[k].w + b3 * orn[k].w;
                y0.x = finish(y0.x, d.nz[0][k].x, d.rs[0][k].x); y0.y = finish(y0.y, d.nz[0][k].y, d.rs[0][k].y);
                y0.z = finish(y0.z, d.nz[0][k].z, d.rs[0][k].z); y0.w = finish(y0.w, d.nz[0][k].w, d.rs[0][k].w);
                y1.x = finish(y1.x, d.nz[1][k].x, d.rs[1][k].x); y1.y = finish(y1.y, d.nz[1][k].y, d.rs[1][k].y);
                y1.z = finish(y1.z, d.nz[1][k].z, d.rs[1][k].z); y1.w = finish(y1.w, d.nz[1][k].w, d.rs[1][k].w);
                if (lane_on) {
                    float* yr = yb + (long)(2 * u) * OW + 4 * (li + 64 * k);
                    *reinterpret_cast<float4*>(yr) = y0;
                    *reinterpret_cast<float4*>(yr + OW) = y1;
                }
            }
        }
#pragma unroll
        for (int k = 0; k < K; ++k) { orA[k] = orB[k]; erB[k] = ern[k]; orB[k] = orn[k]; }
    };
    const int nt = u1 - u0 + 2;
    for (int t = 0; t < nt; t += B) {
#pragma unroll
        for (int j = 0; j < B; ++j) load_step(in[j], u0 - 1 + t + j);
#pragma unroll
        for (int j = 0; j < B; ++j) step(in[j], t + j);
    }
}

struct FirRsParams {
    const float* x; float* y;
    int NC, H, W;
    int R, nseg, LPG, G, nitem;
    float a[4], b[4];
};

template <int K>
__global__ __launch_bounds__(256) void fir_dn2_march_kernel(const FirRsParams p) {
    const int lane = threadIdx.x & 63;
    const int item = blockIdx.x * 4 + (threadIdx.x >> 6);
    if (item >= p.nitem) return;
    const int seg = item % p.nseg, pg = item / p.nseg;
    const int g = lane / p.LPG, li = lane - g * p.LPG;
    const int OH = p.H >> 1, OW = p.W >> 1;
    const int r0 = seg * p.R, r1 = min(r0 + p.R, OH);
    const int plane_raw = pg * p.G + g;
    const bool lane_on = plane_raw < p.NC;
    const int plane = lane_on ? plane_raw : 0;
    const bool grp = K == 1 && p.LPG < 64;
    const bool gfirst = grp && li == 0, glast = grp && li == p.LPG - 1;
    const float* xb = p.x + (long)plane * p.H * p.W + 4 * li;
    float* yb = p.y + (long)plane * OH * OW + 2 * li;
    const float a0 = p.a[0], a1 = p.a[1], a2 = p.a[2], a3 = p.a[3];
    const float b0 = p.b[0], b1 = p.b[1], b2 = p.b[2], b3 = p.b[3];
    auto hrow = [&](int iy, float2 (&h)[K]) __attribute__((always_inline)) {
        const bool ok = iy >= 0 && iy < p.H;
        const float* src = xb + (long)min(max(iy, 0), p.H - 1) * p.W;
        float4 c[K];
#pragma unroll
        for (int k = 0; k < K; ++k) {
            const float4 v = *reinterpret_cast<const float4*>(src + 256 * k);
            c[k].x = ok ? v.x : 0.f; c[k].y = ok ? v.y : 0.f; c[k].z = ok ? v.z : 0.f; c[k].w = ok ? v.w : 0.f;
        }
#pragma unroll
        for (int k = 0; k < K; ++k) {
            float pw = fm_shr1(c[k].w, k > 0 ? fm_lane(c[k - 1].w, 63) : 0.f);
            float nx = fm_shl1(c[k].x, k + 1 < K ? fm_lane(c[k + 1].x, 0) : 0.f);
            pw = gfirst ? 0.f : pw; nx = glast ? 0.f : nx;
            h[k].x = a0 * pw + a1 * c[k].x + a2 * c[k].y + a3 * c[k].z;
            h[k].y = a0 * c[k].y + a1 * c[k].z + a2 * c[k].w + a3 * nx;
        }
    };
    float2 hm1[K], h0[K], h1[K], h2[K];
    hrow(2 * r0 - 1, hm1);
    hrow(2 * r0, h0);
    for (int oy = r0; oy < r1; ++oy) {
        hrow(2 * oy + 1, h1);
        hrow(2 * oy + 2, h2);
#pragma unroll
        for (int k = 0; k < K; ++k) {
            float2 o;
            o.x = b0 * hm1[k].x + b1 * h0[k].x + b2 * h1[k].x + b3 * h2[k].x;
            o.y = b0 * hm1[k].y + b1 * h0[k].y + b2 * h1[k].y + b3 * h2[k].y;
            if (lane_on) *reinterpret_cast<float2*>(yb + (long)oy * OW + 128 * k) = o;
            hm1[k] = h1[k]; h0[k] = h2[k];
        }
    }
}

template <int K>
__global__ __launch_bounds__(256) void fir_up2_march_kernel(const FirRsParams p) {
    const int lane = threadIdx.x & 63;
    const int item = blockIdx.x * 4 + (threadIdx.x >> 6);
    if (item >= p.nitem) return;
    const int seg = item % p.nseg, pg = item / p.nseg;
    const int g = lane / p.LPG, li = lane - g * p.LPG;
    const int OW = 2 * p.W;
    const int u0 = seg * p.R, u1 = min(u0 + p.R, p.H);
    const int plane_raw = pg * p.G + g;
    const bool lane_on = plane_raw < p.NC;
    const int plane = lane_on ? plane_raw : 0;
    const bool grp = K == 1 && p.LPG < 64;
    const bool gfirst = grp && li == 0, glast = grp && li == p.LPG - 1;
    const float* xb = p.x + (long)plane * p.H * p.W + 2 * li;
    float* yb = p.y + (long)plane * (2 * p.H) * OW + 4 * li;
    const float a0 = p.a[0], a1 = p.a[1], a2 = p.a[2], a3 = p.a[3];
    const float b0 = p.b[0], b1 = p.b[1], b2 = p.b[2], b3 = p.b[3];
    auto hrow = [&](int u, float4 (&h)[K]) __attribute__((always_inline)) {
        const bool ok = u >= 0 && u < p.H;
        const float* src = xb + (long)min(max(u, 0), p.H - 1) * p.W;
// ... 39 lines not shown
```

### sh-gan_amd/csrc/upfirdn2d.hip

```cpp
#include "shg_common.h"
#include "fir_march.h"
#include <stdlib.h>

struct UfdParams {
    const float* x;
    const float* f;
    float* y;
    int NC, C, H, W, OH, OW;
    int fh, fw, upx, upy, dnx, dny, px0, py0, flip;
    float gain;
    const float* scale;
    const float* bias;
    const float* noise;
    const float* residual;
    int noise_mode;
    float noise_strength;
    int act;
    float alpha, act_gain, clamp;
    int has_epilogue;
    int pl_ph2, pl_pp;
};

__device__ __forceinline__ float ufd_epilogue(const UfdParams& p, float v, int nc, int oy, int ox) {
    if (!p.has_epilogue) return v;
// ... 466 lines not shown
    p.pl_ph2 = H / 2 + 1; p.pl_pp = PP;
    return ufd_launch(p, (hipStream_t)stream);
}

extern "C" int shg_fir_pad2_sep_supported(int H, int W, int PP) {
    if (H < 2 || W < 8 || W > 512 || !(W % 64 == 0 ? (W == 64 || W == 128 || W == 256 || W == 512) : 64 % W == 0)) return 0;
    if (PP > 0 && (H % 2 || W % 2 || PP % 4 || PP < W / 2 + 1)) return 0;
    return 1;
}

extern "C" int shg_fir_pad2_sep_f32(const float* x, const float* taps_host, float* y, int N, int C, int H, int W, int PP, int flip,
                                    float gain, void* stream) {
    SHG_CHECK_ARG(x && taps_host && y, "fir_pad2_sep: null pointer");
    SHG_CHECK_ARG(N >= 1 && C >= 1, "fir_pad2_sep: bad shape");
    SHG_CHECK_ARG(shg_fir_pad2_sep_supported(H, W, PP), "fir_pad2_sep: unsupported geometry (shg_fir_pad2_sep_supported)");
    SHG_CHECK_ARG((long)N * C * (H + 1) * (W + 1) <= 2147483647L && (PP == 0 || 4L * N * C * (H / 2 + 1) * PP <= 2147483647L),
                  "fir_pad2_sep: tensor too large");
    FirMarchParams p{};
    p.x = x; p.y = y; p.NC = N * C; p.H = H; p.W = W;
    p.mode = PP > 0; p.pitch = PP > 0 ? PP : W + 1; p.ph2 = H / 2 + 1;
    for (int k = 0; k < 4; ++k) {
        p.a[k] = taps_host[flip ? k : 3 - k];
        p.b[k] = taps_host[4 + (flip ? k : 3 - k)] * gain;
    }
    const int OH = H + 1;
    const bool wide = p.mode && W % 256 == 0 && (reinterpret_cast<uintptr_t>(x) & 15) == 0 && (reinterpret_cast<uintptr_t>(y) & 7) == 0 &&
                      PP % 2 == 0;
    p.LPG = wide ? 64 : (W < 64 ? W : 64);
    p.G = wide ? 1 : 64 / p.LPG;
    const int npg = shg_cdiv(p.NC, p.G);
    int nseg = shg_cdiv(8192, npg);
    if (nseg > OH / 16) nseg = OH / 16;
    if (nseg < 1) nseg = 1;
    p.R = shg_cdiv(OH, nseg); p.nseg = shg_cdiv(OH, p.R); p.nitem = npg * p.nseg;
    const dim3 grid(shg_cdiv(p.nitem, 4));
    hipStream_t s = (hipStream_t)stream;
    if (wide) {
        if (W == 256) hipLaunchKernelGGL((fir_down_march4_kernel<1, 8>), grid, dim3(256), 0, s, p);
        else hipLaunchKernelGGL((fir_down_march4_kernel<2, 8>), grid, dim3(256), 0, s, p);
    } else {
        const int K = shg_cdiv(W, 64);
        if (K == 1) hipLaunchKernelGGL((fir_down_march_kernel<1, 8>), grid, dim3(256), 0, s, p);
        else if (K == 2) hipLaunchKernelGGL((fir_down_march_kernel<2, 8>), grid, dim3(256), 0, s, p);
        else if (K == 4) hipLaunchKernelGGL((fir_down_march_kernel<4, 8>), grid, dim3(256), 0, s, p);
        else hipLaunchKernelGGL((fir_down_march_kernel<8, 4>), grid, dim3(256), 0, s, p);
    }
    SHG_CHECK_LAUNCH();
    return SHG_OK;
}

extern "C" int shg_upfir_planar_f32(const float* mid, const float* f, float* y, int N, int C, int H, int W, int flip, float gain,
                                    const float* scale, const float* bias, const float* noise, int noise_mode,
                                    float noise_strength, int act, float alpha, float act_gain, float clamp,
                                    const float* residual, void* stream) {
    SHG_CHECK_ARG(mid && f && y, "upfir_planar: null pointer");
    SHG_CHECK_ARG(N >= 1 && C >= 1 && H >= 1 && W >= 1, "upfir_planar: bad shape");
    SHG_CHECK_ARG(4L * N * C * (H + 1) * (W + 1) <= 2147483647L && 4L * N * C * H * W <= 2147483647L, "upfir_planar: tensor too large");
    SHG_CHECK_ARG(noise_mode >= 0 && noise_mode <= 2, "upfir_planar: bad noise_mode");
    UfdParams p{};
    p.x = mid; p.f = f; p.y = y; p.NC = N * C; p.C = C; p.H = H; p.W = W; p.OH = 2 * H; p.OW = 2 * W;
    p.fh = 4; p.fw = 4; p.upx = p.upy = p.dnx = p.dny = 1; p.px0 = p.py0 = 1; p.flip = flip ? 1 : 0; p.gain = gain;
    p.scale = scale; p.bias = bias; p.noise = noise; p.residual = residual;
    p.noise_mode = noise ? noise_mode : 0; p.noise_strength = noise_strength;
    p.act = act; p.alpha = alpha; p.act_gain = act_gain; p.clamp = clamp; p.has_epilogue = 1;
    const int TV = W >= 96 ? 128 : (W >= 48 ? 64 : 32), TU = 1024 / TV;
    const int tiles = shg_cdiv(W, TV) * shg_cdiv(H, TU);
    int gz = 8192 / tiles; if (gz < 1) gz = 1; if (gz > p.NC) gz = p.NC;
    const bool vec = (W % 2 == 0) && (((uintptr_t)y | (uintptr_t)residual | (uintptr_t)noise) % 16 == 0);
    dim3 grid(shg_cdiv(W, TV), shg_cdiv(H, TU), gz);
    void (*kern)(const UfdParams) =
        TV == 128 ? (vec ? fir_up_planar_kernel<true, 128> : fir_up_planar_kernel<false, 128>)
      : TV == 64  ? (vec ? fir_up_planar_kernel<true, 64> : fir_up_planar_kernel<false, 64>)
                  : (vec ? fir_up_planar_kernel<true, 32> : fir_up_planar_kernel<false, 32>);
    hipLaunchKernelGGL(kern, grid, dim3(256), 0, (hipStream_t)stream, p);
    SHG_CHECK_LAUNCH();
    return SHG_OK;
}

extern "C" int shg_upfir_planar_sep_supported(int H, int W) {
    if (H < 1 || W < 4 || W > 256 || W % 2) return 0;
    return (W >= 128 ? W % 128 == 0 : 64 % (W / 2) == 0) ? 1 : 0;
}

extern "C" int shg_upfir_planar_sep_f32(const float* mid, const float* taps_host, float* y, int N, int C, int H, int W, int flip,
                                        float gain, const float* scale, const float* bias, const float* noise, int noise_mode,
                                        float noise_strength, int act, float alpha, float act_gain, float clamp,
                                        const float* residual, void* stream) {
    SHG_CHECK_ARG(mid && taps_host && y, "upfir_planar_sep: null pointer");
    SHG_CHECK_ARG(N >= 1 && C >= 1, "upfir_planar_sep: bad shape");
    SHG_CHECK_ARG(shg_upfir_planar_sep_supported(H, W), "upfir_planar_sep: unsupported geometry (shg_upfir_planar_sep_supported)");
    SHG_CHECK_ARG(4L * N * C * (H + 1) * (W + 1) <= 2147483647L && 4L * N * C * H * W <= 2147483647L, "upfir_planar_sep: tensor too large");
    SHG_CHECK_ARG(noise_mode >= 0 && noise_mode <= 2, "upfir_planar_sep: bad noise_mode");
    SHG_CHECK_ARG((((uintptr_t)y | (uintptr_t)residual | (uintptr_t)noise) & 15) == 0, "upfir_planar_sep: y / residual / noise must be 16-byte aligned");
    FirUpParams p{};
    p.mid = mid; p.y = y; p.scale = scale; p.bias = bias; p.noise = noise; p.residual = residual;
    p.NC = N * C; p.C = C; p.H = H; p.W = W;
    p.noise_mode = noise ? noise_mode : 0; p.noise_strength = noise_strength;
    p.act = act; p.alpha = alpha; p.act_gain = act_gain; p.clamp = clamp;
    for (int k = 0; k < 4; ++k) {
        p.a[k] = taps_host[flip ? k : 3 - k];
        p.b[k] = taps_host[4 + (flip ? k : 3 - k)] * gain;
    }
    p.LPG = W / 2 < 64 ? W / 2 : 64; p.G = 64 / p.LPG;
    const int npg = shg_cdiv(p.NC, p.G);
    int nseg = shg_cdiv(8192, npg);
    if (nseg > H / 8) nseg = H / 8;
    if (nseg < 1) nseg = 1;
    p.R = shg_cdiv(H, nseg); p.nseg = shg_cdiv(H, p.R); p.nitem = npg * p.nseg;
    const dim3 grid(shg_cdiv(p.nitem, 4));
    hipStream_t s = (hipStream_t)stream;
    if (W <= 128) hipLaunchKernelGGL((fir_up_march_kernel<1, 2>), grid, dim3(256), 0, s, p);
    else hipLaunchKernelGGL((fir_up_march_kernel<2, 1>), grid, dim3(256), 0, s, p);
    SHG_CHECK_LAUNCH();
    return SHG_OK;
}

extern "C" int shg_fir_resample2_sep_supported(int H, int W, int up) {
    if (up == 1) return (H >= 2 && H % 2 == 0 && W >= 8 && W % 4 == 0 && (W <= 256 ? 64 % (W / 4) == 0 : W == 512)) ? 1 : 0;
    if (up == 2) return (H >= 1 && W >= 4 && W % 2 == 0 && (W <= 128 ? 64 % (W / 2) == 0 : W == 256)) ? 1 : 0;
    return 0;
}

extern "C" int shg_fir_resample2_sep_f32(const float* x, const float* taps_host, float* y, int N, int C, int H, int W, int up, int flip,
                                         float gain, void* stream) {
    SHG_CHECK_ARG(x && taps_host && y, "fir_resample2_sep: null pointer");
    SHG_CHECK_ARG(N >= 1 && C >= 1, "fir_resample2_sep: bad shape");
    SHG_CHECK_ARG(shg_fir_resample2_sep_supported(H, W, up), "fir_resample2_sep: unsupported geometry (shg_fir_resample2_sep_supported)");
    SHG_CHECK_ARG((long)N * C * H * W * (up == 2 ? 4 : 1) <= 2147483647L, "fir_resample2_sep: tensor too large");
    SHG_CHECK_ARG((((uintptr_t)x | (uintptr_t)y) & 15) == 0, "fir_resample2_sep: x / y must be 16-byte aligned");
    FirRsParams p{};
    p.x = x; p.y = y; p.NC = N * C; p.H = H; p.W = W;
    for (int k = 0; k < 4; ++k) {
        p.a[k] = taps_host[flip ? k : 3 - k];
        p.b[k] = taps_host[4 + (flip ? k : 3 - k)] * gain;
    }
    const int lanes = up == 1 ? W / 4 : W / 2;
    p.LPG = lanes < 64 ? lanes : 64; p.G = 64 / p.LPG;
    const int K = shg_cdiv(lanes, 64);
    const int npg = shg_cdiv(p.NC, p.G);
    const int rows = up == 1 ? H / 2 : H;
    int nseg = shg_cdiv(8192, npg);
    if (nseg > rows / 8) nseg = rows / 8;
    if (nseg < 1) nseg = 1;
    p.R = shg_cdiv(rows, nseg); p.nseg = shg_cdiv(rows, p.R); p.nitem = npg * p.nseg;
    const dim3 grid(shg_cdiv(p.nitem, 4));
    hipStream_t s = (hipStream_t)stream;
    if (up == 1) {
        if (K == 1) hipLaunchKernelGGL((fir_dn2_march_kernel<1>), grid, dim3(256), 0, s, p);
        else hipLaunchKernelGGL((fir_dn2_march_kernel<2>), grid, dim3(256), 0, s, p);
    } else {
        if (K == 1) hipLaunchKernelGGL((fir_up2_march_kernel<1>), grid, dim3(256), 0, s, p);
        else hipLaunchKernelGGL((fir_up2_march_kernel<2>), grid, dim3(256), 0, s, p);
    }
    SHG_CHECK_LAUNCH();
    return SHG_OK;
}
```

### sh-gan_amd/kernels.py

```python
import contextlib
import ctypes
import math

import torch

from . import _lib
from ._lib import check

SQRT2 = math.sqrt(2.0)
_NULLCTX = contextlib.nullcontext()


class _Launch:
    __slots__ = ('dev', 'keep', '_ctx')

    def __init__(self):
        self.dev = None
        self.keep = []
        self._ctx = None

    def _own(self, t, name):
        if self.dev is None:
            self.dev = t.device
        elif t.device != self.dev:
# ... 490 lines not shown
    def __init__(self, wt, wsq, o, i, op, kh, kw, groups=1, w=None, wscale=None, flip=False):
        self.wt, self.wsq, self.o, self.i, self.op, self.kh, self.kw, self.groups = wt, wsq, o, i, op, kh, kw, groups
        self.wu, self.wu4, self.wu_up, self.wu_down, self._w, self._wscale, self._flip = None, None, None, None, w, wscale, flip

    def _poly(self, entry):
        if self._w is None or self.groups != 1 or self.kh != 3 or self.kw != 3:
            raise _lib.ShgError('PreppedWeight: polyphase forms need an ungrouped 3x3 weight')
        L = _Launch()
        w, ws = L.req(self._w, 'w'), L.req(self._wscale, 'wscale')
        size = (self.op // 64) * ((self.i + 7) // 8) * 16 * 64 * 8
        wa, wb = L.new((size,)), L.new((size,))
        with L:
            check(getattr(_lib.get_lib(), entry)(_ptr(w), _ptr(ws), _ptr(wa), _ptr(wb), self.o, self.i, self.op,
                                                 int(bool(self._flip)), L.stream()), entry)
        return wa, wb

    def down_poly(self):
        if self.wu_down is None:
            self.wu_down = self._poly('shg_conv_weight_prep_down_poly_f32')
        return self.wu_down

    def up_poly(self):
        if self.wu_up is None:
            self.wu_up = self._poly('shg_conv_weight_prep_up_poly_f32')
        return self.wu_up

    def wino(self):
        if self.wu is None:
            if self._w is None or self.groups != 1 or self.kh != 3 or self.kw != 3:
                raise _lib.ShgError('PreppedWeight.wino: needs an ungrouped 3x3 weight')
            L = _Launch()
            w, ws = L.req(self._w, 'w'), L.req(self._wscale, 'wscale')
            kc = int(_lib.get_lib().shg_conv_wino_chunk())
            nchunk = (self.i + kc - 1) // kc
            self.wu = L.new(((self.op // 64) * nchunk * 16 * 64 * kc,))
            with L:
                check(_lib.get_lib().shg_conv_weight_prep_wino_f32(_ptr(w), _ptr(ws), _ptr(self.wu), self.o, self.i, self.op,
                                                                   int(bool(self._flip)), L.stream()), 'conv_weight_prep_wino')
        return self.wu

    def wino4(self):
        if self.wu4 is None:
            if self._w is None or self.groups != 1 or self.kh != 3 or self.kw != 3:
                raise _lib.ShgError('PreppedWeight.wino4: needs an ungrouped 3x3 weight')
            L = _Launch()
            w, ws = L.req(self._w, 'w'), L.req(self._wscale, 'wscale')
            self.wu4 = L.new((int(_lib.get_lib().shg_conv_wino4_weight_elems(self.op, self.i)),))
            with L:
                check(_lib.get_lib().shg_conv_weight_prep_wino4_f32(_ptr(w), _ptr(ws), _ptr(self.wu4), self.o, self.i, self.op,
                                                                    int(bool(self._flip)), L.stream()), 'conv_weight_prep_wino4')
        return self.wu4


def conv_weight_prep(w, demod=False, gain=1.0, flip=False, groups=1):
    L = _Launch()
    w = L.req(w, 'w')
    o_all, i, kh, kw = w.shape
    o = o_all // groups
    op = (o + 63) // 64 * 64
    kk = kh * kw
    ip = (i + 31) // 32 * 32
    wt = L.new((groups, ip * kk * op))
    wsq = L.new((groups, i * op)) if demod else None
    wscale = L.new((o,))
    lib = _lib.get_lib()
    with L:
        for g in range(groups):
            wg = w[g * o:(g + 1) * o]
            check(lib.shg_conv_weight_prep_f32(_ptr(wg), _ptr(wt[g]), _ptr(wscale), _ptr(wsq[g]) if demod else None, o, i, kh, kw,
                                               op, int(bool(demod)), float(gain), int(bool(flip)), L.stream()), 'conv_weight_prep')
    keep = groups == 1 and kh == 3 and kw == 3
    return PreppedWeight(wt, wsq, o, i, op, kh, kw, groups, w=w if keep else None, wscale=wscale if keep else None, flip=flip)


WINO = True
WINO_MIN = 16
WINO4 = True
WINO4_MIN = 32
WINO4_U = None
_WINO4_ROUTES = {None: 0, 'reg': 1, 'lds': 2, 'lds_8x64': 3}
WINO_SPLIT = True
UP_POLY = True
DOWN_POLY = True

MODE_SAME, MODE_DOWN2, MODE_UP2T = 0, 1, 2
_CONV_CLASS = {MODE_SAME: 'conv_mfma_s1', MODE_DOWN2: 'conv_mfma_s2', MODE_UP2T: 'conv_mfma_up'}


def _wino_workspace(L, bytes_fn, *shape):
    ws_bytes = int(bytes_fn(*shape)) if WINO_SPLIT else 0
    return (L.new((ws_bytes // 4,)) if ws_bytes else None), ws_bytes


def conv2d(x, pw, mode=MODE_SAME, pad=0, in_scale=None, out_scale=None, bias=None, noise=None, noise_strength=1.0,
           act=False, gain=1.0, alpha=0.2, act_gain=SQRT2, clamp=256.0, residual=None, planar=False):
    L = _Launch()
    x = L.req(x, 'x')
    nb, i, h, w = x.shape
    if i != pw.i:
        raise _lib.ShgError(f'conv2d: x has {i} channels, weights expect {pw.i}')
    L.view(pw.wt, 'weights')
    if mode == MODE_SAME:
        oh, ow = h + 2 * pad - pw.kh + 1, w + 2 * pad - pw.kw + 1
    elif mode == MODE_DOWN2:
        oh, ow = (h + 2 * pad - pw.kh) // 2 + 1, (w + 2 * pad - pw.kw) // 2 + 1
    else:
        oh, ow = 2 * h + 1, 2 * w + 1
    lib = _lib.get_lib()
    if mode == MODE_UP2T and planar:
        y = L.new((4, nb, pw.o, h + 1, w + 1))
    else:
        y = L.new((nb, pw.o, oh, ow))
    noise, nmode = _noise_args(L, noise, nb)
    a, al, g, cl = _act_args(act, gain, alpha, act_gain, clamp)
    residual = L.req(residual, 'residual')
    in_scale, out_scale, bias = L.req(in_scale, 'in_scale'), L.req(out_scale, 'out_scale'), L.req(bias, 'bias')
    if residual is not None and tuple(residual.shape) != tuple(y.shape):
        raise _lib.ShgError('conv2d: residual shape mismatch')
    tail_al = (_addr(noise) or 0) | (_addr(residual) or 0)
    if (WINO and mode == MODE_SAME and pad == 1 and pw.kh == 3 and pw.kw == 3 and pw.groups == 1 and h >= WINO_MIN and w >= WINO_MIN
            and w % 4 == 0 and x.data_ptr() % 16 == 0 and tail_al % 8 == 0 and i <= 1024 and (pw.wu is not None or pw._w is not None)):
        direct = 2.0 * nb * pw.o * i * 9 * oh * ow
        if WINO4 and h >= WINO4_MIN and tail_al % 16 == 0 and lib.shg_conv2d_wino4_supported(nb, i, pw.o, h, w):
            wu = pw.wino4()
            executed = 2.0 * nb * pw.o * i * 36.0 * ((h + 3) // 4) * ((w + 3) // 4)
            ws, ws_bytes = _wino_workspace(L, lib.shg_conv2d_wino4_workspace_bytes, nb, i, pw.o, pw.op, h, w)
            with _timed(L, 'conv_wino4', direct, executed):
                check(lib.shg_conv2d_wino4_route_f32(
                    _ptr(x), _ptr(wu), _ptr(y), nb, i, pw.o, pw.op, h, w, _ptr(in_scale), _ptr(out_scale), _ptr(bias), _ptr(noise),
                    nmode, float(noise_strength), a, al, g, cl, _ptr(residual), _WINO4_ROUTES[WINO4_U], _ptr(ws), ws_bytes, L.stream()),
                    'conv2d_wino4')
            return y
        wu = pw.wino()
        ws, ws_bytes = _wino_workspace(L, lib.shg_conv2d_wino_workspace_bytes, nb, i, pw.o, pw.op, h, w)
        with _timed(L, 'conv_wino', direct, direct * 16.0 / 36.0):
            check(lib.shg_conv2d_wino_ws_f32(
                _ptr(x), _ptr(wu), _ptr(y), nb, i, pw.o, pw.op, h, w, _ptr(in_scale), _ptr(out_scale), _ptr(bias), _ptr(noise), nmode,
                float(noise_strength), a, al, g, cl, _ptr(residual), _ptr(ws), ws_bytes, L.stream()), 'conv2d_wino')
        return y
    if (UP_POLY and mode == MODE_UP2T and planar and pw.groups == 1 and pw._w is not None and out_scale is None and bias is None
            and noise is None and residual is None and not act and gain == 1.0 and x.data_ptr() % 16 == 0
            and lib.shg_conv2d_up_poly_supported(nb, i, pw.o, h, w)):
        wa, wb = pw.up_poly()
        nba, nbb = ((h + 1 + 2) // 3) * ((w + 1 + 2) // 3), (h // 2) * (w // 2)
        executed = 2.0 * nb * pw.o * i * (16.0 * (nba + nbb) + h + w)
        ws, ws_bytes = _wino_workspace(L, lib.shg_conv2d_up_poly_workspace_bytes, nb, i, pw.o, pw.op, h, w)
        with _timed(L, 'conv_poly_up', 2.0 * nb * pw.o * i * 9 * h * w, executed):
            check(lib.shg_conv2d_up_poly_ws_f32(_ptr(x), _ptr(pw.wt), _ptr(wa), _ptr(wb), _ptr(y), nb, i, pw.o, pw.op, h, w,
                                                _ptr(in_scale), _ptr(ws), ws_bytes, L.stream()), 'conv2d_up_poly')
        return y
    ws, ws_bytes = None, 0
    if mode != MODE_UP2T or planar:
        ws_bytes = int(lib.shg_conv2d_workspace_bytes(nb, i, pw.o, h, w, pw.kh, pw.kw, mode, pad, pw.groups))
        if ws_bytes:
            ws = L.new((ws_bytes // 4,))
    pix = (h * w) if mode == MODE_UP2T else (oh * ow)
    with _timed(L, _CONV_CLASS[mode] if pw.kh == 3 else 'conv_mfma_1x1', 2.0 * nb * pw.o * i * pw.kh * pw.kw * pix):
        check(lib.shg_conv2d_f32(
            _ptr(x), _ptr(pw.wt), _ptr(y), nb, i, pw.o, pw.op, h, w, pw.kh, pw.kw, mode, pad, pw.groups, pw.wt.shape[1],
            _ptr(in_scale), _ptr(out_scale), _ptr(bias), _ptr(noise), nmode, float(noise_strength), a, al, g, cl, _ptr(residual),
            1 if planar else 0, _ptr(ws), ws_bytes, L.stream()), 'conv2d')
    return y


DOWN_POLY_MIN_I, DOWN_POLY_MIN_OUT = 128, 32


def down_poly_supported(x, pw, force=False):
    n, i, h, w = x.shape
    if not force and (i < DOWN_POLY_MIN_I or min(h, w) // 2 < DOWN_POLY_MIN_OUT):
        return False
    return bool(DOWN_POLY and pw.groups == 1 and pw.kh == 3 and pw.kw == 3 and pw._w is not None and h % 2 == 0 and w % 2 == 0
                and x.is_cuda and _lib.get_lib().shg_conv2d_down_poly_supported(n, i, pw.o, h // 2, w // 2))


def fir_conv_down2(x, f, pw, bias=None, act=False, gain=1.0, alpha=0.2, act_gain=SQRT2, clamp=256.0, residual=None, flip_filter=False):
    L = _Launch()
    x, f = L.req(x, 'x'), L.req(f, 'f')
    if tuple(f.shape) != (4, 4):
        raise _lib.ShgError('fir_conv_down2: f must be 4x4')
    n, i, h, w = x.shape
    oh, ow = h // 2, w // 2
    lib = _lib.get_lib()
    pp4 = (ow + 1 + 3) // 4 * 4
    taps = sep_taps(f) if lib.shg_fir_pad2_sep_supported(h, w, pp4) else None
    pp = (ow + 1 + 31) // 32 * 32 if (taps is not None and w % 256 == 0) else pp4
    wa, wb = pw.down_poly()
    L.view(wa, 'weights')
    xp = L.new((4, n, i, oh + 1, pp))
    y = L.new((n, pw.o, oh, ow))
    bias, residual = L.req(bias, 'bias'), L.req(residual, 'residual')
    if residual is not None and tuple(residual.shape) != tuple(y.shape):
        raise _lib.ShgError('fir_conv_down2: residual shape mismatch')
    a, al, g, cl = _act_args(act, gain, alpha, act_gain, clamp)
    with _timed(L, 'upfirdn2d', 4.0 * (x.numel() + n * i * (h + 1) * (w + 1))):
        if taps is not None:
            check(lib.shg_fir_pad2_sep_f32(_ptr(x), taps, _ptr(xp), n, i, h, w, pp, int(bool(flip_filter)), 1.0, L.stream()), 'fir_pad2_sep')
        else:
            check(lib.shg_fir_down_planar_f32(_ptr(x), _ptr(f), _ptr(xp), n, i, h, w, pp, int(bool(flip_filter)), 1.0, L.stream()),
                  'fir_down_planar')
    nba, nbb = ((oh + 2) // 3) * ((ow + 2) // 3), (oh // 2) * (ow // 2)
    with _timed(L, 'conv_poly_down', 2.0 * n * pw.o * i * 9 * oh * ow, 2.0 * n * pw.o * i * 16.0 * (nba + nbb)):
        check(lib.shg_conv2d_down_poly_f32(_ptr(xp), _ptr(wa), _ptr(wb), _ptr(y), n, i, pw.o, pw.op, oh, ow, pp, None, _ptr(bias),
                                           a, al, g, cl, _ptr(residual), L.stream()), 'conv2d_down_poly')
    return y


def upfir_planar(mid, f, scale=None, bias=None, noise=None, noise_strength=1.0, residual=None, act=False, gain=1.0,
                 alpha=0.2, act_gain=SQRT2, clamp=256.0, fir_gain=4.0, flip=False):
    L = _Launch()
    mid = L.req(mid, 'mid')
    f = L.req(f, 'f')
    if mid.ndim != 5 or mid.shape[0] != 4 or tuple(f.shape) != (4, 4):
        raise _lib.ShgError('upfir_planar: mid must be [4,N,C,H+1,W+1] and f 4x4')
    _, n, c, hp, wp = mid.shape
    h, w = hp - 1, wp - 1
    y = L.new((n, c, 2 * h, 2 * w))
    noise, nmode = _noise_args(L, noise, n)
    a, al, g, cl = _act_args(act, gain, alpha, act_gain, clamp)
    residual = L.req(residual, 'residual')
    scale, bias = L.req(scale, 'scale'), L.req(bias, 'bias')
    if residual is not None and tuple(residual.shape) != tuple(y.shape):
        raise _lib.ShgError('upfir_planar: residual shape mismatch')
    with _timed(L, 'fir_up_planar', 4.0 * (mid.numel() + y.numel() * (2 if residual is not None else 1))):
        lib = _lib.get_lib()
        taps = sep_taps(f) if lib.shg_upfir_planar_sep_supported(h, w) else None
        if taps is not None and all(t is None or t.data_ptr() % 16 == 0 for t in (y, noise, residual)):
            check(lib.shg_upfir_planar_sep_f32(_ptr(mid), taps, _ptr(y), n, c, h, w, int(bool(flip)), float(fir_gain),
                                               _ptr(scale), _ptr(bias), _ptr(noise), nmode, float(noise_strength), a, al, g, cl,
                                               _ptr(residual), L.stream()), 'upfir_planar_sep')
        else:
            check(lib.shg_upfir_planar_f32(_ptr(mid), _ptr(f), _ptr(y), n, c, h, w, int(bool(flip)), float(fir_gain),
                                           _ptr(scale), _ptr(bias), _ptr(noise), nmode, float(noise_strength), a, al, g, cl,
                                           _ptr(residual), L.stream()), 'upfir_planar')
    return y


def conv1x1_thin_in(x, w, bias=None, wgain=1.0, act=True, gain=1.0, alpha=0.2, act_gain=SQRT2, clamp=256.0):
    L = _Launch()
    x = L.req(x, 'x')
    w = L.req(w, 'w')
    bias = L.req(bias, 'bias')
    n, i, h, wd = x.shape
    o = w.shape[0]
    y = L.new((n, o, h, wd))
    a, al, g, cl = _act_args(act, gain, alpha, act_gain, clamp)
    with _timed(L, 'fromrgb', 4.0 * (x.numel() + y.numel())):
        check(_lib.get_lib().shg_conv1x1_thin_in_f32(_ptr(x), _ptr(w), _ptr(bias), _ptr(y), n, i, o, h * wd, float(wgain), a, al, g,
                                                     cl, L.stream()), 'conv1x1_thin_in')
    return y


def torgb(x, w, styles=None, bias=None, base_up=None, f=None):
    L = _Launch()
    x = L.req(x, 'x')
    w = L.req(w, 'w')
    styles, bias, base_up, f = L.req(styles, 'styles'), L.req(bias, 'bias'), L.req(base_up, 'base_up'), L.req(f, 'f')
    n, i, h, wd = x.shape
    o = w.shape[0]
    y = L.new((n, o, h, wd))
    with _timed(L, 'torgb', 4.0 * (x.numel() + y.numel() + (base_up.numel() if base_up is not None else 0))):
        check(_lib.get_lib().shg_torgb_f32(_ptr(x), _ptr(w), _ptr(styles), _ptr(bias), _ptr(base_up), _ptr(f), _ptr(y), n, i, o, h,
                                           wd, L.stream()), 'torgb')
    return y



def dense(x, w, b=None, wgain=1.0, bgain=1.0, act=False, gain=1.0, alpha=0.2, act_gain=SQRT2, clamp=256.0, out=None):
    L = _Launch()
    x = L.req(x, 'x')
    w = L.req(w, 'w')
    b = L.req(b, 'b')
    n, k = x.shape
    o = w.shape[0]
    if w.shape[1] != k:
        raise _lib.ShgError(f'dense: x has {k} features, weight expects {w.shape[1]}')
    y = L.rows(out, 'out') if out is not None else L.new((n, o))
    a, al, g, cl = _act_args(act, gain, alpha, act_gain, clamp)
    with _timed(L, 'dense', 4.0 * (w.numel() + x.numel() + n * o)):
        check(_lib.get_lib().shg_dense_f32(_ptr(x), _ptr(w), _ptr(b), _ptr(y), n, k, o, x.stride(0), y.stride(0), float(wgain),
                                           float(bgain), a, al, g, cl, L.stream()), 'dense')
    return y


def demod_weight(w, prenorm=False):
    L = _Launch()
    w = L.req(w, 'w')
    o, i = w.shape[0], w.shape[1]
    k = w.numel() // (o * i)
    wn, wsq, sfac = torch.empty_like(w), L.new((o, i)), L.new((o,))
    with L:
        check(_lib.get_lib().shg_demod_weight_f32(_ptr(w), _ptr(wn), _ptr(wsq), _ptr(sfac), o, i, k, int(bool(prenorm)), L.stream()), 'demod_weight')
    return wn, wsq, sfac


def demod_weight_backward(wn, sfac, gwn, gwsq):
    L = _Launch()
    wn, sfac, gwn, gwsq = L.req(wn, 'wn'), L.req(sfac, 'sfac'), L.req(gwn, 'gwn'), L.req(gwsq, 'gwsq')
    o, i = wn.shape[0], wn.shape[1]
    k = wn.numel() // (o * i)
    gw = torch.empty_like(wn)
    with L:
        check(_lib.get_lib().shg_demod_weight_backward_f32(_ptr(wn), _ptr(sfac), _ptr(gwn), _ptr(gwsq), _ptr(gw), o, i, k, L.stream()),
              'demod_weight_backward')
    return gw


def style_factors_supported(styles, wsq):
    n, i = styles.shape
    return (styles.is_cuda and styles.dtype == torch.float32 and styles.ndim == 2 and wsq is not None and wsq.ndim == 2 and wsq.shape[1] == i
# ... 280 lines not shown
```

### sh-gan_amd/model_zoo/stylegan.py

```python
import math

import os

import numpy as np
import torch
import torch.nn as nn

from .. import kernels
from .common import utils
from .common.get_model import get_model, register
from .stylegan_utils import grad_ops, conv2d_gradfix, conv2d_resample, fma, misc, upfirdn2d

version = '0'
symbol = 'stylegan'



def _make_act(activation):
    return None if activation is None else utils.get_unit()(activation)()


def _act_kwargs(act_obj, gain=1.0):
    if act_obj is None:
        return dict(act=False, gain=gain)
# ... 98 lines not shown
        if self.padding_mode != 'zeros' or self.groups != 1 or tuple(self.dilation) != (1, 1):
            raise NotImplementedError('conv2d: only zero padding, groups=1, dilation=1 run on the HIP path')
        stride, pad = self.stride[0], self.padding[0]
        if grad_ops.wants_grad(x, self.weight, self.bias):
            from .stylegan_utils import conv2d_gradfix
            y = conv2d_gradfix.conv2d(x, self.weight * self.weight_gain, None if self.bias is None else self.bias * self.bias_gain,
                                      stride=stride, padding=pad)
            return torch.relu(y) if relu else y
        mode = kernels.MODE_SAME if stride == 1 else kernels.MODE_DOWN2
        b = self.bias.detach() if self.bias is not None else None
        return kernels.conv2d(x, self.prepped(), mode=mode, pad=pad, bias=b, act=relu, alpha=0.0, act_gain=1.0, clamp=None)


class dense(nn.Module):

    def __init__(self, in_features, out_features, bias=True, bias_init=0, activation=None, lr_multi=1):
        super().__init__()
        self.activation = _make_act(activation)
        self.weight = nn.Parameter(torch.randn([out_features, in_features]) / lr_multi)
        self.bias = nn.Parameter(torch.full([out_features], np.float32(bias_init))) if bias else None
        self.weight_gain = lr_multi / np.sqrt(in_features)
        self.bias_gain = lr_multi
        self.lr_multi, self.bias_init = lr_multi, bias_init
        self.repr = 'dense({}, {}, bias={}, act={}, lr_multi={})'.format(in_features, out_features, bias, activation, lr_multi)

    def forward(self, x, out=None):
        if grad_ops.wants_grad(x, self.weight, self.bias):
            if x.ndim == 2 and x.dtype == torch.float32:
                from .stylegan_utils import dense_ops
                y = dense_ops.linear(x, self.weight, self.bias, self.weight_gain, self.bias_gain)
                ak = _act_kwargs(self.activation)
                if ak is None:
                    return self.activation(y)
                return grad_ops.bias_act(y, None, **ak) if ak['act'] or ak.get('gain', 1.0) != 1.0 else y
            y = x.matmul((self.weight * self.weight_gain).t())
            ak = _act_kwargs(self.activation)
            b = None if self.bias is None else self.bias * self.bias_gain
            if ak is None:
                return self.activation(y if b is None else y + b)
            return grad_ops.bias_act(y, b, **ak)
        ak = _act_kwargs(self.activation)
        b = self.bias.detach() if self.bias is not None else None
        if ak is None:
            return self.activation(kernels.dense(x, self.weight.detach(), b, wgain=self.weight_gain, bgain=self.bias_gain))
        return kernels.dense(x, self.weight.detach(), b, wgain=self.weight_gain, bgain=self.bias_gain, out=out, **ak)

    def __repr__(self):
        return self.repr


def modulated_conv2d(x, weight, styles, noise=None, up=1, down=1, padding=0, resample_filter=None, demodulate=True,
                     flip_weight=True, fused_modconv=True, _prepped=None, _epilogue=None, _tail=None):
    batch_size = x.shape[0]
    out_channels, in_channels, kh, kw = weight.shape
    misc.assert_shape(weight, [out_channels, in_channels, kh, kw])
    misc.assert_shape(x, [batch_size, in_channels, None, None])
    misc.assert_shape(styles, [batch_size, in_channels])
    if (fused_modconv and x.dtype == torch.float16 and x.is_cuda and down == 1 and not _epilogue and _tail is None
            and not grad_ops.wants_grad(x, weight, styles, noise)):
        y = _modulated_conv2d_half_infer(x, weight, styles, noise, up, padding, resample_filter, demodulate, flip_weight, None, _act_kwargs(None),
                                         None, fused=True)
        if y is not None:
            return y
    if grad_ops.generic_route(x, weight, styles, noise):
        if _epilogue:
            raise NotImplementedError('modulated_conv2d: the fused epilogue is an inference-path extension')
        return _modulated_conv2d_train(x, weight, styles, noise, up, down, padding, resample_filter, demodulate, flip_weight, _tail)
    ep = dict(_epilogue or {})
    if noise is not None and noise.ndim == 4 and noise.shape[0] == 1:
        noise = noise[0, 0]

    fast_plain = up == 1 and down == 1 and kh == kw and kh in (1, 3) and padding == kh // 2
    fast_up = (up == 2 and down == 1 and kh == kw == 3 and padding == 1 and resample_filter is not None
               and resample_filter.ndim == 2 and tuple(resample_filter.shape) == (4, 4))
    if fast_plain or fast_up:
        pw = _prepped
        if pw is None:
            pw = kernels.conv_weight_prep(weight, demod=demodulate, flip=(flip_weight if fast_up else not flip_weight))
        s, d = kernels.modconv_style_prep(styles, pw, demod=demodulate)
        if fast_plain:
            return kernels.conv2d(x, pw, mode=kernels.MODE_SAME, pad=padding, in_scale=s, out_scale=d, noise=noise,
                                  bias=ep.get('bias'), residual=ep.get('residual'),
                                  **{k: v for k, v in ep.items() if k in ('act', 'gain', 'alpha', 'act_gain', 'clamp')})
        mid = kernels.conv2d(x, pw, mode=kernels.MODE_UP2T, in_scale=s, planar=True)
        return kernels.upfir_planar(mid, resample_filter, scale=d.reshape(-1) if d is not None else None, noise=noise,
                                    bias=ep.get('bias'), residual=ep.get('residual'),
                                    **{k: v for k, v in ep.items() if k in ('act', 'gain', 'alpha', 'act_gain', 'clamp')})

    pw_tmp = kernels.conv_weight_prep(weight, demod=demodulate)
    s, d = kernels.modconv_style_prep(styles, pw_tmp, demod=demodulate)
    wn = weight
    if demodulate:
        wn = weight * weight.square().mean([1, 2, 3], keepdim=True).rsqrt()
    y = conv2d_resample.conv2d_resample(x=kernels.scale_channels(x, s.reshape(-1)), w=wn, f=resample_filter, up=up, down=down,
                                        padding=padding, flip_weight=flip_weight)
    return kernels.bias_act(y, scale=d.reshape(-1) if d is not None else None, noise=noise, bias=ep.get('bias'),
                            residual=ep.get('residual'), act=ep.get('act', False), gain=ep.get('gain', 1.0))


class _DemodWeightFn(torch.autograd.Function):
    @staticmethod
    def forward(ctx, weight, prenorm):
        wn, wsq, sfac = kernels.demod_weight(weight.detach(), prenorm)
        ctx.save_for_backward(wn, sfac, weight)
        ctx.mark_non_differentiable(sfac)
        return wn, wsq, sfac

    @staticmethod
    def backward(ctx, gwn, gwsq, _gs):
        wn, sfac, weight = ctx.saved_tensors
        if torch.is_grad_enabled():
            g = 0
            if gwn is not None:
                g = g + gwn
            if gwsq is not None:
                g = g + 2 * gwsq[:, :, None, None] * wn
            s = weight.square().mean([1, 2, 3], keepdim=True).rsqrt()
            return s * (g - wn * (g * wn).mean([1, 2, 3], keepdim=True)), None
        return kernels.demod_weight_backward(wn, sfac, None if gwn is None else gwn.contiguous(), None if gwsq is None else gwsq.contiguous()), None


FUSED_DEMOD_WEIGHT = os.environ.get('SHG_FUSED_DEMOD', '1') == '1'


def _weight_factors(half, weight, demodulate):
    if (FUSED_DEMOD_WEIGHT and demodulate and weight.is_cuda and weight.dtype == torch.float32 and weight.ndim == 4
            and grad_ops.wants_grad(weight)):
        wn, wsq, _ = _DemodWeightFn.apply(weight.contiguous(), bool(half))
        return wn, wsq
    if half and demodulate:
        o, i, kh, kw = weight.shape
        weight = weight * (1 / np.sqrt(i * kh * kw) / weight.norm(float('inf'), dim=[1, 2, 3], keepdim=True))
    wsq = None
    if demodulate:
        weight = weight * weight.square().mean([1, 2, 3], keepdim=True).rsqrt()
        wsq = weight.square().sum([2, 3])
    return weight, wsq


def _style_factors_composed(half, styles, wsq):
    if half:
        styles = styles / styles.norm(float('inf'), dim=1, keepdim=True)
    styles = styles * styles.square().mean().rsqrt()
    if styles.is_cuda and styles.dtype == torch.float32 and styles.ndim == 2:
        from .stylegan_utils import dense_ops
        return styles, (dense_ops.nt(styles.square(), wsq) + 1e-8).rsqrt()
    return styles, (styles.square().matmul(wsq.t()) + 1e-8).rsqrt()


class _StyleFactorsFn(torch.autograd.Function):
    @staticmethod
    def forward(ctx, styles, wsq, half):
        sn, d, aux = kernels.style_factors(styles.detach(), wsq.detach(), half)
        ctx.save_for_backward(styles, wsq, sn, d, aux)
        ctx.half = half
        return sn, d

    @staticmethod
    def backward(ctx, gsn, gd):
        styles, wsq, sn, d, aux = ctx.saved_tensors
        if torch.is_grad_enabled() and CLOSED_STYLE_FACTORS_BACKWARD:
            gs, gw = _StyleFactorsBwdFn.apply(styles, wsq, gsn, gd, sn, d, aux, ctx.half)
            return (gs if ctx.needs_input_grad[0] else None), (gw if ctx.needs_input_grad[1] else None), None
        if torch.is_grad_enabled():
            with torch.enable_grad():
                s_in = styles if styles.requires_grad else styles.detach().requires_grad_(True)
                w_in = wsq if wsq.requires_grad else wsq.detach().requires_grad_(True)
# ... 284 lines not shown
                                                   wgain=self.weight_gain, **ak)
                return kernels.conv2d(x, self.prepped(), mode=kernels.MODE_SAME, pad=self.padding, bias=b, **ak)
            f = self.resample_filter
            fw, fh = f.shape[1], f.shape[0]
            p = self.padding
            pads = [p + (fw - 1) // 2, p + (fw - 2) // 2, p + (fh - 1) // 2, p + (fh - 2) // 2]
            if tuple(f.shape) == (4, 4) and p == 1 and kernels.down_poly_supported(x, self.prepped()):
                return kernels.fir_conv_down2(x, f, self.prepped(), bias=b, **ak)
            y = kernels.upfirdn2d(x, f, padx0=pads[0], padx1=pads[1], pady0=pads[2], pady1=pads[3])
            return kernels.conv2d(y, self.prepped(), mode=kernels.MODE_DOWN2, pad=0, bias=b, **ak)
        w = self.weight.detach() * self.weight_gain
        y = conv2d_resample.conv2d_resample(x=x, w=w, f=self.resample_filter, up=self.up, down=self.down,
                                            padding=self.padding, flip_weight=(self.up == 1))
        if ak is None:
            if b is not None:
                y = kernels.bias_act(y, bias=b, act=False)
            return self.activation(y, gain=gain)
        return kernels.bias_act(y, bias=b, **ak)

    def __repr__(self):
        return self.repr


class synthesis_layer(conv2d_layer):

    def __init__(self, in_channels, out_channels, kernel_size, w_dim, resolution, bias=True,
                 activation='lrelu_agc(alpha=0.2, gain=sqrt_2)', up=1, resample_filter=[1, 3, 3, 1], use_noise=True):
        super().__init__(in_channels, out_channels, kernel_size, bias=bias, activation=activation, up=up, down=1,
                         resample_filter=resample_filter)
        self.affine = dense(w_dim, in_channels, bias=True, bias_init=1, activation=None)
        self.resolution = resolution
        self.use_noise = use_noise
        if use_noise:
            self.register_buffer('noise_const', torch.randn([resolution, resolution]))
            self.noise_strength = nn.Parameter(torch.zeros([]))
        self.bias = nn.Parameter(torch.zeros([out_channels]))
        self.repr = 'synthesis_layer({}, {}, kernal_size={}, bias={}, up={}, act={}, noise={})'.format(
            in_channels, out_channels, kernel_size, bias, up, activation, use_noise)

    def prepped(self):
        return _cache_of(self).get('w', [self.weight], lambda: kernels.conv_weight_prep(self.weight.detach(), demod=True))

    def _noise_strength_host(self):
        return _cache_of(self).get('ns', [self.noise_strength], lambda: float(self.noise_strength.detach().cpu()))

    def forward(self, x, w, fused_modconv=True, gain=1, noise_mode='random', residual=None, styles_sd=None):
        if noise_mode not in ('random', 'const', 'none'):
            raise AssertionError(f'bad noise_mode {noise_mode!r}')
        noise = None
        if self.use_noise and noise_mode == 'random':
            noise = torch.randn([x.shape[0], 1, self.resolution, self.resolution], device=x.device)
        elif self.use_noise and noise_mode == 'const':
            noise = self.noise_const
        ak = _act_kwargs(self.activation, gain)
        if ak is None or self.up not in (1, 2) or self.weight.shape[2] != 3:
            raise NotImplementedError('synthesis_layer: HIP path needs lrelu_agc, 3x3 kernels and up in {1,2}')
        route = layer_route(self, x, w, self.weight, self.bias, self.affine.weight, residual)
        if route == 'f16_fused':
            y = _modulated_conv2d_half_infer(x, self.weight.detach(), self.affine(w), None if noise is None else noise * self.noise_strength.detach(),
                                             self.up, self.padding, self.resample_filter, True, self.up == 1, self.bias.detach(), ak, residual,
                                             cache=_cache_of(self), fused=bool(fused_modconv))
            if y is not None:
                return y
        if route != 'f32_fused':
            y = modulated_conv2d(x=x, weight=self.weight, styles=self.affine(w), noise=None if noise is None else noise * self.noise_strength,
                                 up=self.up, padding=self.padding, resample_filter=self.resample_filter, flip_weight=(self.up == 1),
                                 _tail=(self.bias, ak))
            return y if residual is None else y + residual
        ns = 0.0
        if noise is not None:
            if x.is_cuda and torch.cuda.is_current_stream_capturing():
                noise, ns = noise * self.noise_strength.detach(), 1.0
            else:
                ns = self._noise_strength_host()
        pw = self.prepped()
        if styles_sd is not None:
            s, d = styles_sd
        else:
            s, d = kernels.modconv_style_prep(self.affine(w), pw, demod=True)
        b = self.bias.detach()
        if self.up == 1:
            return kernels.conv2d(x, pw, mode=kernels.MODE_SAME, pad=self.padding, in_scale=s, out_scale=d, noise=noise,
                                  noise_strength=ns, bias=b, residual=residual, **ak)
        mid = kernels.conv2d(x, pw, mode=kernels.MODE_UP2T, in_scale=s, planar=True)
        return kernels.upfir_planar(mid, self.resample_filter, scale=d.reshape(-1), noise=noise, noise_strength=ns, bias=b,
                                    residual=residual, **ak)


class torgb_layer(conv2d_layer):

    def __init__(self, in_channels, out_channels, kernel_size, w_dim, activation=None):
        super().__init__(in_channels, out_channels, kernel_size, bias=True, activation=activation, up=1, down=1,
                         resample_filter=None)
        self.affine = dense(w_dim, in_channels, bias=True, bias_init=1, activation=None)

    def forward(self, x, w, fused_modconv=True, base_img=None, base_filter=None, styles_sd=None):
        if self.activation is not None or self.weight.shape[2] != 1 or self.weight.shape[0] > 4:
            raise NotImplementedError('torgb_layer: HIP path is the 1x1, <=4-channel, linear form')
        route = layer_route(self, x, w, self.weight, self.bias, self.affine.weight, base_img)
        if route == 'f16_fused':
            from .. import kernels_f16
            if fused_modconv:
                st = self.affine(w) * self.weight_gain
                ys = [kernels_f16.conv2d(x[j:j + 1], (self.weight.detach() * st[j].reshape(1, -1, 1, 1)).to(torch.float16), self.bias.detach(), 1, 0)
                      for j in range(x.shape[0])]
                y = ys[0] if len(ys) == 1 else torch.cat(ys)
            else:
                y = kernels_f16.conv2d(x, self.weight.detach().to(torch.float16), self.bias.detach(), 1, 0, in_scale=self.affine(w) * self.weight_gain)
            y = y.to(dtype=torch.float32, memory_format=torch.contiguous_format)
            return y if base_img is None else upfirdn2d.upsample2d(base_img, base_filter) + y
        if route != 'f32_fused':
            y = modulated_conv2d(x=x, weight=self.weight, styles=self.affine(w) * self.weight_gain, demodulate=False)
            y = grad_ops.add_channel_bias(y, self.bias)
            y = y.to(dtype=torch.float32, memory_format=torch.contiguous_format)
            return y if base_img is None else upfirdn2d.upsample2d(base_img, base_filter) + y
        if styles_sd is not None:
            s = styles_sd[0]
        else:
            s, _ = kernels.modconv_style_prep(self.affine(w), None, demod=False, pre_gain=self.weight_gain)
        wmat = self.weight.detach().reshape(self.weight.shape[0], -1)
        return kernels.torgb(x, wmat, s, self.bias.detach(), base_up=base_img, f=base_filter)



def normalize_2nd_moment(x, dim=1, eps=1e-8):
    if grad_ops.wants_grad(x):
        return x * (x.square().mean(dim=dim, keepdim=True) + eps).rsqrt()
    if dim != 1 or x.ndim != 2:
        raise NotImplementedError('normalize_2nd_moment: HIP path handles [N,K] along dim 1')
    return kernels.normalize_2nd_moment(x, eps)


@register('stylegan2_mapping', version)
class Mapping(nn.Module):

    def __init__(self, z_dim=512, c_dim=0, w_dim=512, num_ws=14, num_layers=8, embed_features=None, layer_features=None,
                 activation='lrelu_agc(alpha=0.2, gain=sqrt_2, clamp=256)', lr_multiplier=0.01, w_avg_beta=0.995):
        super().__init__()
        self.z_dim, self.c_dim, self.w_dim, self.num_ws = z_dim, c_dim, w_dim, num_ws
        self.num_layers, self.w_avg_beta = num_layers, w_avg_beta
        if embed_features is None:
            embed_features = w_dim
        if c_dim == 0:
            embed_features = 0
        if layer_features is None:
            layer_features = w_dim
        widths = [z_dim + embed_features] + [layer_features] * (num_layers - 1) + [w_dim]
        if c_dim > 0:
            self.embed = dense(c_dim, embed_features)
        for idx in range(num_layers):
            setattr(self, f'fc{idx}', dense(widths[idx], widths[idx + 1], activation=activation, lr_multi=lr_multiplier))
        if num_ws is not None and w_avg_beta is not None:
            self.register_buffer('w_avg', torch.zeros([w_dim]))

    def forward(self, z, c, truncation_psi=1, truncation_cutoff=None, skip_w_avg_update=False):
        x = None
        if self.z_dim > 0:
            x = normalize_2nd_moment(z.to(torch.float32))
        if self.c_dim > 0:
            y = normalize_2nd_moment(self.embed(c.to(torch.float32)))
            x = torch.cat([x, y], dim=1) if x is not None else y
        for idx in range(self.num_layers):
            x = getattr(self, f'fc{idx}')(x)
        if self.w_avg_beta is not None and self.training and not skip_w_avg_update:
            self.w_avg.copy_(x.detach().mean(dim=0).lerp(self.w_avg, self.w_avg_beta))
        if self.num_ws is not None:
            x = x.unsqueeze(1).repeat([1, self.num_ws, 1])
# ... 235 lines not shown
```

Baseline: 816.0.

## Pad up-conv phase planes to aligned pitch for vectorized stores and FIR loads

Adds a row pitch parameter to the polyphase up-conv output planes, so width-256 layers use a pitch rounded up to a multiple of 4 instead of W+1. With an even pitch the poly kernel writes paired f32x2 stores, and the separable up-FIR kernel gets a pitched variant that reads aligned rows. The intent is to remove misaligned scalar global accesses between the two stages. The cost is a slightly larger intermediate buffer, and it adds alignment requirements plus a new PhasePlanes wrapper that both call sites must handle.

```diff
diff --git a/include/shgan_hip.h b/include/shgan_hip.h
--- a/include/shgan_hip.h
+++ b/include/shgan_hip.h
@@ -82,6 +82,11 @@
 int shg_upfir_planar_sep_f32(const float* mid, const float* taps_host, float* y, int N, int C, int H, int W, int flip, float gain,
                              const float* scale, const float* bias, const float* noise, int noise_mode, float noise_strength,
                              int act, float alpha, float act_gain, float clamp, const float* residual, void* stream);
+int shg_upfir_planar_sep_pitch_supported(int H, int W, int PP);
+int shg_upfir_planar_sep_pitch_f32(const float* mid, const float* taps_host, float* y, int N, int C, int H, int W, int PP, int flip,
+                                   float gain, const float* scale, const float* bias, const float* noise, int noise_mode,
+                                   float noise_strength, int act, float alpha, float act_gain, float clamp, const float* residual,
+                                   void* stream);
 int shg_conv_weight_prep_up_poly_f32(const float* w, const float* wscale, float* wu_a, float* wu_b, int O, int I, int OP, int flip,
                                      void* stream);
 int shg_conv2d_up_poly_supported(int NB, int I, int O, int H, int W);
@@ -90,6 +95,10 @@
 size_t shg_conv2d_up_poly_workspace_bytes(int NB, int I, int O, int OP, int H, int W);
 int shg_conv2d_up_poly_ws_f32(const float* x, const float* wt, const float* wu_a, const float* wu_b, float* y, int NB, int I, int O,
                               int OP, int H, int W, const float* in_scale, void* workspace, size_t ws_bytes, void* stream);
+int shg_conv2d_up_poly_pitch_supported(int NB, int I, int O, int H, int W, int PP);
+size_t shg_conv2d_up_poly_workspace_pitch_bytes(int NB, int I, int O, int OP, int H, int W, int PP);
+int shg_conv2d_up_poly_ws_pitch_f32(const float* x, const float* wt, const float* wu_a, const float* wu_b, float* y, int NB, int I, int O,
+                                    int OP, int H, int W, int PP, const float* in_scale, void* workspace, size_t ws_bytes, void* stream);
 int shg_fir_down_planar_f32(const float* x, const float* f, float* y, int N, int C, int H, int W, int PP, int flip, float gain,
                             void* stream);
 int shg_fir_pad2_sep_supported(int H, int W, int PP);
diff --git a/sh-gan_amd/_lib.py b/sh-gan_amd/_lib.py
--- a/sh-gan_amd/_lib.py
+++ b/sh-gan_amd/_lib.py
@@ -96,6 +96,12 @@
     'shg_composite_u8': [c_fp, c_fp, c_fp, c_i, c_i, c_i, c_fp],
     'shg_assemble_input_f32': [c_fp, c_fp, c_fp, c_i, c_i, c_i, c_fp],
     'shg_assemble_input_u8': [c_fp, c_fp, c_fp, c_fp, c_i, c_i, c_i, c_fp],
+    'shg_upfir_planar_sep_pitch_supported': [c_i, c_i, c_i],
+    'shg_upfir_planar_sep_pitch_f32': [c_fp, ctypes.POINTER(c_f), c_fp, c_i, c_i, c_i, c_i, c_i, c_i, c_f, c_fp, c_fp, c_fp, c_i, c_f, c_i, c_f, c_f, c_f,
+                                       c_fp, c_fp],
+    'shg_conv2d_up_poly_pitch_supported': [c_i] * 6,
+    'shg_conv2d_up_poly_ws_pitch_f32': [c_fp, c_fp, c_fp, c_fp, c_fp] + [c_i] * 7 + [c_fp, c_fp, ctypes.c_size_t, c_fp],
+    'shg_conv2d_up_poly_workspace_pitch_bytes': [c_i] * 7,
     'shg_conv_weight_prep_up_poly_f32': [c_fp, c_fp, c_fp, c_fp, c_i, c_i, c_i, c_i, c_fp],
     'shg_conv2d_up_poly_supported': [c_i, c_i, c_i, c_i, c_i],
     'shg_conv2d_up_poly_f32': [c_fp, c_fp, c_fp, c_fp, c_fp, c_i, c_i, c_i, c_i, c_i, c_i, c_fp, c_fp],
@@ -193,6 +199,7 @@
     lib.shg_conv2d_wino_workspace_bytes.restype = ctypes.c_size_t
     lib.shg_conv2d_wino4_workspace_bytes.restype = ctypes.c_size_t
     lib.shg_conv2d_up_poly_workspace_bytes.restype = ctypes.c_size_t
+    lib.shg_conv2d_up_poly_workspace_pitch_bytes.restype = ctypes.c_size_t
     lib.shg_conv2d_wgrad_wino_workspace_bytes.restype = ctypes.c_size_t
     lib.shg_conv2d_wgrad_f16_workspace_bytes.restype = ctypes.c_size_t
     lib.shg_image_metrics_scratch_bytes.restype = ctypes.c_size_t
diff --git a/sh-gan_amd/csrc/conv_wino_poly.hip b/sh-gan_amd/csrc/conv_wino_poly.hip
--- a/sh-gan_amd/csrc/conv_wino_poly.hip
+++ b/sh-gan_amd/csrc/conv_wino_poly.hip
@@ -26,6 +26,7 @@
     float alpha, gain, clamp;
     int cps;
     long part_stride;
+    int YP;
 };
 
 namespace poly {
@@ -281,7 +282,7 @@
     mma(apend[0], apend[1], 1);
 
     float* Mx = Vl;
-    const int PWg = DOWN ? p.W : p.W + 1;
+    const int PWg = DOWN ? p.W : p.YP;
     const long plane = DOWN ? (long)p.H * p.W : (long)(p.H + 1) * PWg;
     const int o_l = tid >> 5, t_l = tid & 31;
     f32x2 pre_part[SCHEME == DB ? 4 : 1][2], pre_res[SCHEME == DB ? 4 : 1][2];
@@ -367,17 +368,26 @@
                 float* yeo = yb + pstride + (long)u0 * PWg + v0;
                 float* yoe = yb + 2 * pstride + (long)u0 * PWg + v0;
                 float* yoo = yb + 3 * pstride + (long)u0 * PWg + v0;
-#pragma unroll
-                for (int cc = 0; cc < 2; ++cc) {
-                    yeo[cc] = m[0 * 2 + cc] + m[1 * 2 + cc];
-                    yeo[PWg + cc] = m[1 * 2 + cc] + m[2 * 2 + cc];
-                }
-#pragma unroll
-                for (int r = 0; r < 2; ++r) {
-                    yoe[r * PWg] = m[6 + r * 3] + m[6 + r * 3 + 1];
-                    yoe[r * PWg + 1] = m[6 + r * 3 + 1] + m[6 + r * 3 + 2];
-                    yoo[r * PWg] = m[12 + r * 2];
-                    yoo[r * PWg + 1] = m[12 + r * 2 + 1];
+                if ((PWg & 1) == 0) {
+#pragma unroll
+                    for (int r = 0; r < 2; ++r) {
+                        *reinterpret_cast<f32x2*>(yeo + r * PWg) = f32x2{m[r * 2] + m[(r + 1) * 2], m[r * 2 + 1] + m[(r + 1) * 2 + 1]};
+                        *reinterpret_cast<f32x2*>(yoe + r * PWg) = f32x2{m[6 + r * 3] + m[6 + r * 3 + 1], m[6 + r * 3 + 1] + m[6 + r * 3 + 2]};
+                        *reinterpret_cast<f32x2*>(yoo + r * PWg) = f32x2{m[12 + r * 2], m[12 + r * 2 + 1]};
+                    }
+                } else {
+#pragma unroll
+                    for (int cc = 0; cc < 2; ++cc) {
+                        yeo[cc] = m[0 * 2 + cc] + m[1 * 2 + cc];
+                        yeo[PWg + cc] = m[1 * 2 + cc] + m[2 * 2 + cc];
+                    }
+#pragma unroll
+                    for (int r = 0; r < 2; ++r) {
+                        yoe[r * PWg] = m[6 + r * 3] + m[6 + r * 3 + 1];
+                        yoe[r * PWg + 1] = m[6 + r * 3 + 1] + m[6 + r * 3 + 2];
+                        yoo[r * PWg] = m[12 + r * 2];
+                        yoo[r * PWg + 1] = m[12 + r * 2 + 1];
+                    }
                 }
             }
         }
@@ -432,7 +442,7 @@
     for (int r = 0; r < 16; ++r) red[wave][r][lane] = acc[r];
     __syncthreads();
     if (!pok) return;
-    const int PWg = p.W + 1;
+    const int PWg = p.YP;
     const long plane = (long)(p.H + 1) * PWg;
     const long pix = col ? (long)pos * PWg + p.W : (long)p.H * PWg + pos;
     float* yb = p.y + blockIdx.y * p.part_stride + (long)(col ? 2 : 1) * p.NB * p.O * plane + (long)n * p.O * plane + pix;
@@ -579,27 +589,38 @@
     return wide ? 4 : 5;
 }
 
-extern "C" size_t shg_conv2d_up_poly_workspace_bytes(int NB, int I, int O, int OP, int H, int W) {
-    if (!shg_conv2d_up_poly_supported(NB, I, O, H, W) || OP < 64) return 0;
+extern "C" int shg_conv2d_up_poly_pitch_supported(int NB, int I, int O, int H, int W, int PP) {
+    return (shg_conv2d_up_poly_supported(NB, I, O, H, W) && (PP == W + 1 || (PP > W && PP % 4 == 0))) ? 1 : 0;
+}
+
+extern "C" size_t shg_conv2d_up_poly_workspace_pitch_bytes(int NB, int I, int O, int OP, int H, int W, int PP) {
+    if (!shg_conv2d_up_poly_pitch_supported(NB, I, O, H, W, PP) || OP < 64) return 0;
     PolyParams p{};
     up_poly_plan(p, NB, I, OP, H, W);
-    return shg_wino_split_bytes((long)(p.a.n_ttiles + p.b.n_ttiles) * p.n_otiles, p.nchunk, (size_t)4 * NB * O * (H + 1) * (W + 1) * sizeof(float));
-}
-
-extern "C" int shg_conv2d_up_poly_ws_f32(const float* x, const float* wt, const float* wu_a, const float* wu_b, float* y, int NB, int I,
-                                         int O, int OP, int H, int W, const float* in_scale, void* workspace, size_t ws_bytes, void* stream) {
+    return shg_wino_split_bytes((long)(p.a.n_ttiles + p.b.n_ttiles) * p.n_otiles, p.nchunk, (size_t)4 * NB * O * (H + 1) * PP * sizeof(float));
+}
+
+extern "C" size_t shg_conv2d_up_poly_workspace_bytes(int NB, int I, int O, int OP, int H, int W) {
+    return shg_conv2d_up_poly_workspace_pitch_bytes(NB, I, O, OP, H, W, W + 1);
+}
+
+extern "C" int shg_conv2d_up_poly_ws_pitch_f32(const float* x, const float* wt, const float* wu_a, const float* wu_b, float* y, int NB, int I,
+                                               int O, int OP, int H, int W, int PP, const float* in_scale, void* workspace, size_t ws_bytes,
+                                               void* stream) {
     SHG_CHECK_ARG(x && wt && wu_a && wu_b && y, "conv2d_up_poly: null pointer");
-    SHG_CHECK_ARG(shg_conv2d_up_poly_supported(NB, I, O, H, W), "conv2d_up_poly: unsupported geometry (use shg_conv2d_f32 mode 2)");
+    SHG_CHECK_ARG(shg_conv2d_up_poly_pitch_supported(NB, I, O, H, W, PP), "conv2d_up_poly: unsupported geometry (use shg_conv2d_f32 mode 2)");
     SHG_CHECK_ARG(OP % 64 == 0 && OP >= O, "conv2d_up_poly: OP must be a multiple of 64 and >= O");
-    SHG_CHECK_ARG((long)NB * I * H * W < 2147483647L && 4L * NB * O * (H + 1) * (W + 1) < 2147483647L, "conv2d_up_poly: tensor too large");
+    SHG_CHECK_ARG((long)NB * I * H * W < 2147483647L && 4L * NB * O * (H + 1) * PP < 2147483647L, "conv2d_up_poly: tensor too large");
     SHG_CHECK_ARG((reinterpret_cast<uintptr_t>(x) & 15) == 0, "conv2d_up_poly: x must be 16-byte aligned");
+    SHG_CHECK_ARG(PP % 4 != 0 || (reinterpret_cast<uintptr_t>(y) & 15) == 0, "conv2d_up_poly: planes with an aligned pitch must be 16-byte aligned");
     hipStream_t s = (hipStream_t)stream;
     PolyParams p{};
     p.x = x; p.y = y; p.in_scale = in_scale;
-    p.NB = NB; p.I = I; p.O = O; p.OP = OP; p.H = H; p.W = W;
+    p.NB = NB; p.I = I; p.O = O; p.OP = OP; p.H = H; p.W = W; p.YP = PP;
     p.a.wu = wu_a; p.b.wu = wu_b; p.wt = wt;
     const int variant = up_poly_plan(p, NB, I, OP, H, W);
-    const int ks = shg_wino_split((long)(p.a.n_ttiles + p.b.n_ttiles) * p.n_otiles, p.nchunk, (size_t)4 * NB * O * (H + 1) * (W + 1) * sizeof(float),
+    const size_t out_bytes = (size_t)4 * NB * O * (H + 1) * PP * sizeof(float);
+    const int ks = shg_wino_split((long)(p.a.n_ttiles + p.b.n_ttiles) * p.n_otiles, p.nchunk, out_bytes,
                                   workspace, ws_bytes, shg_addr(workspace) | shg_addr(y), &p.y, &p.cps, &p.part_stride);
     const dim3 grid((p.a.n_ttiles + p.b.n_ttiles) * p.n_otiles + shg_cdiv(p.n_strip_tiles, 4), ks);
     if (variant == 0) hipLaunchKernelGGL((conv_poly_up_kernel<8, 8, 0, 8, 8>), grid, dim3(poly::NT), 0, s, p);
@@ -610,10 +631,15 @@
     else hipLaunchKernelGGL((conv_poly_up_kernel<8, 8, 0, 4, 16>), grid, dim3(poly::NT), 0, s, p);
     SHG_CHECK_LAUNCH();
     if (ks > 1) {
-        shg_launch_wino_split_reduce((const float*)workspace, y, ks, 4 * NB, O, H + 1, W + 1, nullptr, nullptr, nullptr, 0, 0.f, 0, 0.f, 1.f, -1.f, nullptr, s);
+        shg_launch_wino_split_reduce((const float*)workspace, y, ks, 4 * NB, O, H + 1, PP, nullptr, nullptr, nullptr, 0, 0.f, 0, 0.f, 1.f, -1.f, nullptr, s);
         SHG_CHECK_LAUNCH();
     }
     return SHG_OK;
+}
+
+extern "C" int shg_conv2d_up_poly_ws_f32(const float* x, const float* wt, const float* wu_a, const float* wu_b, float* y, int NB, int I,
+                                         int O, int OP, int H, int W, const float* in_scale, void* workspace, size_t ws_bytes, void* stream) {
+    return shg_conv2d_up_poly_ws_pitch_f32(x, wt, wu_a, wu_b, y, NB, I, O, OP, H, W, W + 1, in_scale, workspace, ws_bytes, stream);
 }
 
 extern "C" int shg_conv2d_up_poly_f32(const float* x, const float* wt, const float* wu_a, const float* wu_b, float* y, int NB, int I,
diff --git a/sh-gan_amd/csrc/fir_march.h b/sh-gan_amd/csrc/fir_march.h
--- a/sh-gan_amd/csrc/fir_march.h
+++ b/sh-gan_amd/csrc/fir_march.h
@@ -222,6 +222,7 @@
     const float* mid; float* y;
     const float* scale; const float* bias; const float* noise; const float* residual;
     int NC, C, H, W;
+    int PP;
     int noise_mode;
     float noise_strength;
     int act; float alpha, act_gain, clamp;
@@ -237,122 +238,14 @@
 
 template <int K, int B>
 __global__ __launch_bounds__(256) void fir_up_march_kernel(const FirUpParams p) {
-    const int lane = threadIdx.x & 63;
-    const int item = blockIdx.x * 4 + (threadIdx.x >> 6);
-    if (item >= p.nitem) return;
-    const int seg = item % p.nseg, pg = item / p.nseg;
-    const int g = lane / p.LPG, li = lane - g * p.LPG;
-    const int u0 = seg * p.R, u1 = min(u0 + p.R, p.H);
-    const int plane_raw = pg * p.G + g;
-    const bool lane_on = plane_raw < p.NC;
-    const int plane = lane_on ? plane_raw : 0;
-    const bool grp = K == 1 && p.LPG < 64;
-    const bool gfirst = grp && li == 0, glast = grp && li == p.LPG - 1;
-    const int PW = p.W + 1, OW = 2 * p.W, OH = 2 * p.H;
-    const long P = (long)(p.H + 1) * PW;
-    const float* mb = p.mid + (long)plane * P + 2 * li;
-    const long qs = (long)p.NC * P;
-    const int n = plane / p.C, ch = plane - n * p.C;
-    const float sc = p.scale ? p.scale[plane] : 1.f, bs = p.bias ? p.bias[ch] : 0.f;
-    const float* nzb = p.noise_mode == 0 ? nullptr : (p.noise_mode == 1 ? p.noise : p.noise + (long)n * OH * OW);
-    const float* rsb = p.residual ? p.residual + (long)plane * OH * OW : nullptr;
-    float* yb = p.y + (long)plane * OH * OW;
-    const float a0 = p.a[0], a1 = p.a[1], a2 = p.a[2], a3 = p.a[3];
-    const float b0 = p.b[0], b1 = p.b[1], b2 = p.b[2], b3 = p.b[3];
-
-    struct Row { float e0[2][K], e1[2][K], o0[2][K], o1[2][K], ew[2]; float4 nz[2][K], rs[2][K]; };
-    Row in[B];
-    float4 orA[K], erB[K], orB[K];
-#pragma unroll
-    for (int k = 0; k < K; ++k) orA[k] = erB[k] = orB[k] = make_float4(0.f, 0.f, 0.f, 0.f);
-
-    auto load_step = [&](Row& d, int r) __attribute__((always_inline)) {
-        const int rc = min(max(r, 0), p.H);
-        const float* src = mb + (long)rc * PW;
-#pragma unroll
-        for (int a = 0; a < 2; ++a) {
-            const float* se = src + (2 * a) * qs;
-            const float* so = se + qs;
-#pragma unroll
-            for (int k = 0; k < K; ++k) {
-                d.e0[a][k] = se[128 * k]; d.e1[a][k] = se[128 * k + 1];
-                d.o0[a][k] = so[128 * k]; d.o1[a][k] = so[128 * k + 1];
-            }
-            d.ew[a] = se[p.W - 2 * li];
-        }
-        const int yc = min(max(2 * (r - 1), 0), OH - 2);
-#pragma unroll
-        for (int dy = 0; dy < 2; ++dy)
-#pragma unroll
-            for (int k = 0; k < K; ++k) {
-                const long off = (long)(yc + dy) * OW + 4 * (li + 64 * k);
-                d.nz[dy][k] = nzb ? *reinterpret_cast<const float4*>(nzb + off) : make_float4(0.f, 0.f, 0.f, 0.f);
-                d.rs[dy][k] = rsb ? *reinterpret_cast<const float4*>(rsb + off) : make_float4(0.f, 0.f, 0.f, 0.f);
-            }
-    };
-    auto hfilt = [&](const Row& d, int a, bool ok, float4 (&h)[K]) __attribute__((always_inline)) {
-        float e0[K], e1[K], o0[K], o1[K];
-#pragma unroll
-        for (int k = 0; k < K; ++k) {
-            e0[k] = ok ? d.e0[a][k] : 0.f; e1[k] = ok ? d.e1[a][k] : 0.f;
-            o0[k] = ok ? d.o0[a][k] : 0.f; o1[k] = ok ? d.o1[a][k] : 0.f;
-        }
-        const float ew = ok ? d.ew[a] : 0.f;
-#pragma unroll
-        for (int k = 0; k < K; ++k) {
-            const float fo = k > 0 ? fm_lane(o1[k - 1], 63) : 0.f;
-            float om1 = fm_shr1(o1[k], fo);
-            float e2 = k + 1 < K ? fm_shl1(e0[k], fm_lane(e0[k + 1], 0)) : fm_shl1(e0[k], ew);
-            float o2 = fm_shl1(o0[k], k + 1 < K ? fm_lane(o0[k + 1], 0) : 0.f);
-            om1 = gfirst ? 0.f : om1; e2 = glast ? ew : e2; o2 = glast ? 0.f : o2;
-            h[k].x = a0 * om1 + a1 * e0[k] + a2 * o0[k] + a3 * e1[k];
-            h[k].y = a0 * e0[k] + a1 * o0[k] + a2 * e1[k] + a3 * o1[k];
-            h[k].z = a0 * o0[k] + a1 * e1[k] + a2 * o1[k] + a3 * e2;
-            h[k].w = a0 * e1[k] + a1 * o1[k] + a2 * e2 + a3 * o2;
-        }
-    };
-    auto finish = [&](float v, float nz, float rs) __attribute__((always_inline)) {
-        return fm_act(v * sc + nz * p.noise_strength + bs, p.act, p.alpha, p.act_gain, p.clamp) + rs;
-    };
-    auto step = [&](const Row& d, int t) __attribute__((always_inline)) {
-        const int r = u0 - 1 + t;
-        float4 ern[K], orn[K];
-        hfilt(d, 0, r >= 0 && r <= p.H, ern);
-        hfilt(d, 1, r >= 0 && r <= p.H - 1, orn);
-        const int u = r - 1;
-        if (t >= 2 && u < u1) {
-#pragma unroll
-            for (int k = 0; k < K; ++k) {
-                float4 y0, y1;
-                y0.x = b0 * orA[k].x + b1 * erB[k].x + b2 * orB[k].x + b3 * ern[k].x;
-                y0.y = b0 * orA[k].y + b1 * erB[k].y + b2 * orB[k].y + b3 * ern[k].y;
-                y0.z = b0 * orA[k].z + b1 * erB[k].z + b2 * orB[k].z + b3 * ern[k].z;
-                y0.w = b0 * orA[k].w + b1 * erB[k].w + b2 * orB[k].w + b3 * ern[k].w;
-                y1.x = b0 * erB[k].x + b1 * orB[k].x + b2 * ern[k].x + b3 * orn[k].x;
-                y1.y = b0 * erB[k].y + b1 * orB[k].y + b2 * ern[k].y + b3 * orn[k].y;
-                y1.z = b0 * erB[k].z + b1 * orB[k].z + b2 * ern[k].z + b3 * orn[k].z;
-                y1.w = b0 * erB[k].w + b1 * orB[k].w + b2 * ern[k].w + b3 * orn[k].w;
-                y0.x = finish(y0.x, d.nz[0][k].x, d.rs[0][k].x); y0.y = finish(y0.y, d.nz[0][k].y, d.rs[0][k].y);
-                y0.z = finish(y0.z, d.nz[0][k].z, d.rs[0][k].z); y0.w = finish(y0.w, d.nz[0][k].w, d.rs[0][k].w);
-                y1.x = finish(y1.x, d.nz[1][k].x, d.rs[1][k].x); y1.y = finish(y1.y, d.nz[1][k].y, d.rs[1][k].y);
-                y1.z = finish(y1.z, d.nz[1][k].z, d.rs[1][k].z); y1.w = finish(y1.w, d.nz[1][k].w, d.rs[1][k].w);
-                if (lane_on) {
-                    float* yr = yb + (long)(2 * u) * OW + 4 * (li + 64 * k);
-                    *reinterpret_cast<float4*>(yr) = y0;
-                    *reinterpret_cast<float4*>(yr + OW) = y1;
-                }
-            }
-        }
-#pragma unroll
-        for (int k = 0; k < K; ++k) { orA[k] = orB[k]; erB[k] = ern[k]; orB[k] = orn[k]; }
-    };
-    const int nt = u1 - u0 + 2;
-    for (int t = 0; t < nt; t += B) {
-#pragma unroll
-        for (int j = 0; j < B; ++j) load_step(in[j], u0 - 1 + t + j);
-#pragma unroll
-        for (int j = 0; j < B; ++j) step(in[j], t + j);
-    }
+    constexpr bool AL = false;
+#include "fir_up_march_body.inc"
+}
+
+template <int K, int B>
+__global__ __launch_bounds__(256) void fir_up_march_al_kernel(const FirUpParams p) {
+    constexpr bool AL = true;
+#include "fir_up_march_body.inc"
 }
 
 struct FirRsParams {
diff --git a/sh-gan_amd/csrc/fir_up_march_body.inc b/sh-gan_amd/csrc/fir_up_march_body.inc
--- /dev/null
+++ b/sh-gan_amd/csrc/fir_up_march_body.inc
@@ -0,0 +1,122 @@
+    const int lane = threadIdx.x & 63;
+    const int item = blockIdx.x * 4 + (threadIdx.x >> 6);
+    if (item >= p.nitem) return;
+    const int seg = item % p.nseg, pg = item / p.nseg;
+    const int g = lane / p.LPG, li = lane - g * p.LPG;
+    const int u0 = seg * p.R, u1 = min(u0 + p.R, p.H);
+    const int plane_raw = pg * p.G + g;
+    const bool lane_on = plane_raw < p.NC;
+    const int plane = lane_on ? plane_raw : 0;
+    const bool grp = K == 1 && p.LPG < 64;
+    const bool gfirst = grp && li == 0, glast = grp && li == p.LPG - 1;
+    const int PW = p.PP, OW = 2 * p.W, OH = 2 * p.H;
+    const long P = (long)(p.H + 1) * PW;
+    const float* mb = p.mid + (long)plane * P + 2 * li;
+    const long qs = (long)p.NC * P;
+    const int n = plane / p.C, ch = plane - n * p.C;
+    const float sc = p.scale ? p.scale[plane] : 1.f, bs = p.bias ? p.bias[ch] : 0.f;
+    const float* nzb = p.noise_mode == 0 ? nullptr : (p.noise_mode == 1 ? p.noise : p.noise + (long)n * OH * OW);
+    const float* rsb = p.residual ? p.residual + (long)plane * OH * OW : nullptr;
+    float* yb = p.y + (long)plane * OH * OW;
+    const float a0 = p.a[0], a1 = p.a[1], a2 = p.a[2], a3 = p.a[3];
+    const float b0 = p.b[0], b1 = p.b[1], b2 = p.b[2], b3 = p.b[3];
+
+    struct Row { float e0[2][K], e1[2][K], o0[2][K], o1[2][K], ew[2]; float4 nz[2][K], rs[2][K]; };
+    Row in[B];
+    float4 orA[K], erB[K], orB[K];
+#pragma unroll
+    for (int k = 0; k < K; ++k) orA[k] = erB[k] = orB[k] = make_float4(0.f, 0.f, 0.f, 0.f);
+
+    auto load_step = [&](Row& d, int r) __attribute__((always_inline)) {
+        const int rc = min(max(r, 0), p.H);
+        const float* src = mb + (long)rc * PW;
+#pragma unroll
+        for (int a = 0; a < 2; ++a) {
+            const float* se = src + (2 * a) * qs;
+            const float* so = se + qs;
+#pragma unroll
+            for (int k = 0; k < K; ++k) {
+                if constexpr (AL) {
+                    const float2 e = *reinterpret_cast<const float2*>(se + 128 * k), o = *reinterpret_cast<const float2*>(so + 128 * k);
+                    d.e0[a][k] = e.x; d.e1[a][k] = e.y;
+                    d.o0[a][k] = o.x; d.o1[a][k] = o.y;
+                } else {
+                    d.e0[a][k] = se[128 * k]; d.e1[a][k] = se[128 * k + 1];
+                    d.o0[a][k] = so[128 * k]; d.o1[a][k] = so[128 * k + 1];
+                }
+            }
+            d.ew[a] = se[p.W - 2 * li];
+        }
+        const int yc = min(max(2 * (r - 1), 0), OH - 2);
+#pragma unroll
+        for (int dy = 0; dy < 2; ++dy)
+#pragma unroll
+            for (int k = 0; k < K; ++k) {
+                const long off = (long)(yc + dy) * OW + 4 * (li + 64 * k);
+                d.nz[dy][k] = nzb ? *reinterpret_cast<const float4*>(nzb + off) : make_float4(0.f, 0.f, 0.f, 0.f);
+                d.rs[dy][k] = rsb ? *reinterpret_cast<const float4*>(rsb + off) : make_float4(0.f, 0.f, 0.f, 0.f);
+            }
+    };
+    auto hfilt = [&](const Row& d, int a, bool ok, float4 (&h)[K]) __attribute__((always_inline)) {
+        float e0[K], e1[K], o0[K], o1[K];
+#pragma unroll
+        for (int k = 0; k < K; ++k) {
+            e0[k] = ok ? d.e0[a][k] : 0.f; e1[k] = ok ? d.e1[a][k] : 0.f;
+            o0[k] = ok ? d.o0[a][k] : 0.f; o1[k] = ok ? d.o1[a][k] : 0.f;
+        }
+        const float ew = ok ? d.ew[a] : 0.f;
+#pragma unroll
+        for (int k = 0; k < K; ++k) {
+            const float fo = k > 0 ? fm_lane(o1[k - 1], 63) : 0.f;
+            float om1 = fm_shr1(o1[k], fo);
+            float e2 = k + 1 < K ? fm_shl1(e0[k], fm_lane(e0[k + 1], 0)) : fm_shl1(e0[k], ew);
+            float o2 = fm_shl1(o0[k], k + 1 < K ? fm_lane(o0[k + 1], 0) : 0.f);
+            om1 = gfirst ? 0.f : om1; e2 = glast ? ew : e2; o2 = glast ? 0.f : o2;
+            h[k].x = a0 * om1 + a1 * e0[k] + a2 * o0[k] + a3 * e1[k];
+            h[k].y = a0 * e0[k] + a1 * o0[k] + a2 * e1[k] + a3 * o1[k];
+            h[k].z = a0 * o0[k] + a1 * e1[k] + a2 * o1[k] + a3 * e2;
+            h[k].w = a0 * e1[k] + a1 * o1[k] + a2 * e2 + a3 * o2;
+        }
+    };
+    auto finish = [&](float v, float nz, float rs) __attribute__((always_inline)) {
+        return fm_act(v * sc + nz * p.noise_strength + bs, p.act, p.alpha, p.act_gain, p.clamp) + rs;
+    };
+    auto step = [&](const Row& d, int t) __attribute__((always_inline)) {
+        const int r = u0 - 1 + t;
+        float4 ern[K], orn[K];
+        hfilt(d, 0, r >= 0 && r <= p.H, ern);
+        hfilt(d, 1, r >= 0 && r <= p.H - 1, orn);
+        const int u = r - 1;
+        if (t >= 2 && u < u1) {
+#pragma unroll
+            for (int k = 0; k < K; ++k) {
+                float4 y0, y1;
+                y0.x = b0 * orA[k].x + b1 * erB[k].x + b2 * orB[k].x + b3 * ern[k].x;
+                y0.y = b0 * orA[k].y + b1 * erB[k].y + b2 * orB[k].y + b3 * ern[k].y;
+                y0.z = b0 * orA[k].z + b1 * erB[k].z + b2 * orB[k].z + b3 * ern[k].z;
+                y0.w = b0 * orA[k].w + b1 * erB[k].w + b2 * orB[k].w + b3 * ern[k].w;
+                y1.x = b0 * erB[k].x + b1 * orB[k].x + b2 * ern[k].x + b3 * orn[k].x;
+                y1.y = b0 * erB[k].y + b1 * orB[k].y + b2 * ern[k].y + b3 * orn[k].y;
+                y1.z = b0 * erB[k].z + b1 * orB[k].z + b2 * ern[k].z + b3 * orn[k].z;
+                y1.w = b0 * erB[k].w + b1 * orB[k].w + b2 * ern[k].w + b3 * orn[k].w;
+                y0.x = finish(y0.x, d.nz[0][k].x, d.rs[0][k].x); y0.y = finish(y0.y, d.nz[0][k].y, d.rs[0][k].y);
+                y0.z = finish(y0.z, d.nz[0][k].z, d.rs[0][k].z); y0.w = finish(y0.w, d.nz[0][k].w, d.rs[0][k].w);
+                y1.x = finish(y1.x, d.nz[1][k].x, d.rs[1][k].x); y1.y = finish(y1.y, d.nz[1][k].y, d.rs[1][k].y);
+                y1.z = finish(y1.z, d.nz[1][k].z, d.rs[1][k].z); y1.w = finish(y1.w, d.nz[1][k].w, d.rs[1][k].w);
+                if (lane_on) {
+                    float* yr = yb + (long)(2 * u) * OW + 4 * (li + 64 * k);
+                    *reinterpret_cast<float4*>(yr) = y0;
+                    *reinterpret_cast<float4*>(yr + OW) = y1;
+                }
+            }
+        }
+#pragma unroll
+        for (int k = 0; k < K; ++k) { orA[k] = orB[k]; erB[k] = ern[k]; orB[k] = orn[k]; }
+    };
+    const int nt = u1 - u0 + 2;
+    for (int t = 0; t < nt; t += B) {
+#pragma unroll
+        for (int j = 0; j < B; ++j) load_step(in[j], u0 - 1 + t + j);
+#pragma unroll
+        for (int j = 0; j < B; ++j) step(in[j], t + j);
+    }
diff --git a/sh-gan_amd/csrc/upfirdn2d.hip b/sh-gan_amd/csrc/upfirdn2d.hip
--- a/sh-gan_amd/csrc/upfirdn2d.hip
+++ b/sh-gan_amd/csrc/upfirdn2d.hip
@@ -572,19 +572,25 @@
     return (W >= 128 ? W % 128 == 0 : 64 % (W / 2) == 0) ? 1 : 0;
 }
 
-extern "C" int shg_upfir_planar_sep_f32(const float* mid, const float* taps_host, float* y, int N, int C, int H, int W, int flip,
-                                        float gain, const float* scale, const float* bias, const float* noise, int noise_mode,
-                                        float noise_strength, int act, float alpha, float act_gain, float clamp,
-                                        const float* residual, void* stream) {
+extern "C" int shg_upfir_planar_sep_pitch_supported(int H, int W, int PP) {
+    return (shg_upfir_planar_sep_supported(H, W) && (PP == W + 1 || (PP > W && PP % 4 == 0))) ? 1 : 0;
+}
+
+extern "C" int shg_upfir_planar_sep_pitch_f32(const float* mid, const float* taps_host, float* y, int N, int C, int H, int W, int PP, int flip,
+                                              float gain, const float* scale, const float* bias, const float* noise, int noise_mode,
+                                              float noise_strength, int act, float alpha, float act_gain, float clamp,
+                                              const float* residual, void* stream) {
     SHG_CHECK_ARG(mid && taps_host && y, "upfir_planar_sep: null pointer");
     SHG_CHECK_ARG(N >= 1 && C >= 1, "upfir_planar_sep: bad shape");
-    SHG_CHECK_ARG(shg_upfir_planar_sep_supported(H, W), "upfir_planar_sep: unsupported geometry (shg_upfir_planar_sep_supported)");
-    SHG_CHECK_ARG(4L * N * C * (H + 1) * (W + 1) <= 2147483647L && 4L * N * C * H * W <= 2147483647L, "upfir_planar_sep: tensor too large");
+    SHG_CHECK_ARG(shg_upfir_planar_sep_pitch_supported(H, W, PP), "upfir_planar_sep: unsupported geometry (shg_upfir_planar_sep_pitch_supported)");
+    SHG_CHECK_ARG(4L * N * C * (H + 1) * PP <= 2147483647L && 4L * N * C * H * W <= 2147483647L, "upfir_planar_sep: tensor too large");
     SHG_CHECK_ARG(noise_mode >= 0 && noise_mode <= 2, "upfir_planar_sep: bad noise_mode");
     SHG_CHECK_ARG((((uintptr_t)y | (uintptr_t)residual | (uintptr_t)noise) & 15) == 0, "upfir_planar_sep: y / residual / noise must be 16-byte aligned");
+    const bool al = PP % 4 == 0;
+    SHG_CHECK_ARG(!al || ((uintptr_t)mid & 15) == 0, "upfir_planar_sep: planes with an aligned pitch must be 16-byte aligned");
     FirUpParams p{};
     p.mid = mid; p.y = y; p.scale = scale; p.bias = bias; p.noise = noise; p.residual = residual;
-    p.NC = N * C; p.C = C; p.H = H; p.W = W;
+    p.NC = N * C; p.C = C; p.H = H; p.W = W; p.PP = PP;
     p.noise_mode = noise ? noise_mode : 0; p.noise_strength = noise_strength;
     p.act = act; p.alpha = alpha; p.act_gain = act_gain; p.clamp = clamp;
     for (int k = 0; k < 4; ++k) {
@@ -599,10 +605,23 @@
     p.R = shg_cdiv(H, nseg); p.nseg = shg_cdiv(H, p.R); p.nitem = npg * p.nseg;
     const dim3 grid(shg_cdiv(p.nitem, 4));
     hipStream_t s = (hipStream_t)stream;
-    if (W <= 128) hipLaunchKernelGGL((fir_up_march_kernel<1, 2>), grid, dim3(256), 0, s, p);
-    else hipLaunchKernelGGL((fir_up_march_kernel<2, 1>), grid, dim3(256), 0, s, p);
+    if (W <= 128) {
+        if (al) hipLaunchKernelGGL((fir_up_march_al_kernel<1, 2>), grid, dim3(256), 0, s, p);
+        else hipLaunchKernelGGL((fir_up_march_kernel<1, 2>), grid, dim3(256), 0, s, p);
+    } else {
+        if (al) hipLaunchKernelGGL((fir_up_march_al_kernel<2, 1>), grid, dim3(256), 0, s, p);
+        else hipLaunchKernelGGL((fir_up_march_kernel<2, 1>), grid, dim3(256), 0, s, p);
+    }
     SHG_CHECK_LAUNCH();
     return SHG_OK;
+}
+
+extern "C" int shg_upfir_planar_sep_f32(const float* mid, const float* taps_host, float* y, int N, int C, int H, int W, int flip,
+                                        float gain, const float* scale, const float* bias, const float* noise, int noise_mode,
+                                        float noise_strength, int act, float alpha, float act_gain, float clamp,
+                                        const float* residual, void* stream) {
+    return shg_upfir_planar_sep_pitch_f32(mid, taps_host, y, N, C, H, W, W + 1, flip, gain, scale, bias, noise, noise_mode, noise_strength, act,
+                                          alpha, act_gain, clamp, residual, stream);
 }
 
 extern "C" int shg_fir_resample2_sep_supported(int H, int W, int up) {
diff --git a/sh-gan_amd/kernels.py b/sh-gan_amd/kernels.py
--- a/sh-gan_amd/kernels.py
+++ b/sh-gan_amd/kernels.py
@@ -596,6 +596,26 @@
 WINO_SPLIT = True
 UP_POLY = True
 DOWN_POLY = True
+UP_PITCH = None
+UP_PITCH_SHIPPED = {256: 4}
+
+
+class PhasePlanes:
+    __slots__ = ('t', 'w')
+
+    def __init__(self, t, w):
+        self.t, self.w = t, w
+
+
+def up_plane_pitch(h, w):
+    if UP_PITCH not in (None, 'dense', 'pad4', 'pad32'):
+        raise _lib.ShgError(f'UP_PITCH: unknown layout {UP_PITCH!r}')
+    q = {None: UP_PITCH_SHIPPED.get(w), 'dense': None, 'pad4': 4, 'pad32': 32}[UP_PITCH]
+    if q is None:
+        return w + 1
+    pp = (w + 1 + q - 1) // q * q
+    return pp if _lib.get_lib().shg_upfir_planar_sep_pitch_supported(h, w, pp) else w + 1
+
 
 MODE_SAME, MODE_DOWN2, MODE_UP2T = 0, 1, 2
 _CONV_CLASS = {MODE_SAME: 'conv_mfma_s1', MODE_DOWN2: 'conv_mfma_s2', MODE_UP2T: 'conv_mfma_up'}
@@ -621,8 +641,12 @@
     else:
         oh, ow = 2 * h + 1, 2 * w + 1
     lib = _lib.get_lib()
+    poly_up = (UP_POLY and mode == MODE_UP2T and planar and pw.groups == 1 and pw._w is not None and out_scale is None and bias is None
+               and noise is None and residual is None and not act and gain == 1.0 and x.data_ptr() % 16 == 0
+               and lib.shg_conv2d_up_poly_supported(nb, i, pw.o, h, w))
+    pp = up_plane_pitch(h, w) if poly_up and planar == 'pitch' else w + 1
     if mode == MODE_UP2T and planar:
-        y = L.new((4, nb, pw.o, h + 1, w + 1))
+        y = L.new((4, nb, pw.o, h + 1, pp))
     else:
         y = L.new((nb, pw.o, oh, ow))
     noise, nmode = _noise_args(L, noise, nb)
@@ -652,17 +676,19 @@
                 _ptr(x), _ptr(wu), _ptr(y), nb, i, pw.o, pw.op, h, w, _ptr(in_scale), _ptr(out_scale), _ptr(bias), _ptr(noise), nmode,
                 float(noise_strength), a, al, g, cl, _ptr(residual), _ptr(ws), ws_bytes, L.stream()), 'conv2d_wino')
         return y
-    if (UP_POLY and mode == MODE_UP2T and planar and pw.groups == 1 and pw._w is not None and out_scale is None and bias is None
-            and noise is None and residual is None and not act and gain == 1.0 and x.data_ptr() % 16 == 0
-            and lib.shg_conv2d_up_poly_supported(nb, i, pw.o, h, w)):
+    if poly_up:
         wa, wb = pw.up_poly()
         nba, nbb = ((h + 1 + 2) // 3) * ((w + 1 + 2) // 3), (h // 2) * (w // 2)
         executed = 2.0 * nb * pw.o * i * (16.0 * (nba + nbb) + h + w)
-        ws, ws_bytes = _wino_workspace(L, lib.shg_conv2d_up_poly_workspace_bytes, nb, i, pw.o, pw.op, h, w)
+        ws, ws_bytes = _wino_workspace(L, lib.shg_conv2d_up_poly_workspace_pitch_bytes, nb, i, pw.o, pw.op, h, w, pp)
         with _timed(L, 'conv_poly_up', 2.0 * nb * pw.o * i * 9 * h * w, executed):
-            check(lib.shg_conv2d_up_poly_ws_f32(_ptr(x), _ptr(pw.wt), _ptr(wa), _ptr(wb), _ptr(y), nb, i, pw.o, pw.op, h, w,
-                                                _ptr(in_scale), _ptr(ws), ws_bytes, L.stream()), 'conv2d_up_poly')
-        return y
+            if pp == w + 1:
+                check(lib.shg_conv2d_up_poly_ws_f32(_ptr(x), _ptr(pw.wt), _ptr(wa), _ptr(wb), _ptr(y), nb, i, pw.o, pw.op, h, w,
+                                                    _ptr(in_scale), _ptr(ws), ws_bytes, L.stream()), 'conv2d_up_poly')
+            else:
+                check(lib.shg_conv2d_up_poly_ws_pitch_f32(_ptr(x), _ptr(pw.wt), _ptr(wa), _ptr(wb), _ptr(y), nb, i, pw.o, pw.op, h, w, pp,
+                                                          _ptr(in_scale), _ptr(ws), ws_bytes, L.stream()), 'conv2d_up_poly_pitch')
+        return y if pp == w + 1 else PhasePlanes(y, w)
     ws, ws_bytes = None, 0
     if mode != MODE_UP2T or planar:
         ws_bytes = int(lib.shg_conv2d_workspace_bytes(nb, i, pw.o, h, w, pw.kh, pw.kw, mode, pad, pw.groups))
@@ -723,12 +749,13 @@
 def upfir_planar(mid, f, scale=None, bias=None, noise=None, noise_strength=1.0, residual=None, act=False, gain=1.0,
                  alpha=0.2, act_gain=SQRT2, clamp=256.0, fir_gain=4.0, flip=False):
     L = _Launch()
+    mid, w = (mid.t, mid.w) if isinstance(mid, PhasePlanes) else (mid, None)
     mid = L.req(mid, 'mid')
     f = L.req(f, 'f')
     if mid.ndim != 5 or mid.shape[0] != 4 or tuple(f.shape) != (4, 4):
         raise _lib.ShgError('upfir_planar: mid must be [4,N,C,H+1,W+1] and f 4x4')
-    _, n, c, hp, wp = mid.shape
-    h, w = hp - 1, wp - 1
+    _, n, c, hp, pp = mid.shape
+    h, w = hp - 1, (pp - 1 if w is None else w)
     y = L.new((n, c, 2 * h, 2 * w))
     noise, nmode = _noise_args(L, noise, n)
     a, al, g, cl = _act_args(act, gain, alpha, act_gain, clamp)
@@ -736,10 +763,16 @@
     scale, bias = L.req(scale, 'scale'), L.req(bias, 'bias')
     if residual is not None and tuple(residual.shape) != tuple(y.shape):
         raise _lib.ShgError('upfir_planar: residual shape mismatch')
-    with _timed(L, 'fir_up_planar', 4.0 * (mid.numel() + y.numel() * (2 if residual is not None else 1))):
+    with _timed(L, 'fir_up_planar', 4.0 * (4 * n * c * (h + 1) * (w + 1) + y.numel() * (2 if residual is not None else 1))):
         lib = _lib.get_lib()
         taps = sep_taps(f) if lib.shg_upfir_planar_sep_supported(h, w) else None
-        if taps is not None and all(t is None or t.data_ptr() % 16 == 0 for t in (y, noise, residual)):
+        if pp != w + 1:
+            if taps is None or not all(t is None or t.data_ptr() % 16 == 0 for t in (mid, y, noise, residual)):
+                raise _lib.ShgError('upfir_planar: padded phase planes need a separable filter and 16-byte aligned operands')
+            check(lib.shg_upfir_planar_sep_pitch_f32(_ptr(mid), taps, _ptr(y), n, c, h, w, pp, int(bool(flip)), float(fir_gain),
+                                                     _ptr(scale), _ptr(bias), _ptr(noise), nmode, float(noise_strength), a, al, g, cl,
+                                                     _ptr(residual), L.stream()), 'upfir_planar_sep_pitch')
+        elif taps is not None and all(t is None or t.data_ptr() % 16 == 0 for t in (y, noise, residual)):
             check(lib.shg_upfir_planar_sep_f32(_ptr(mid), taps, _ptr(y), n, c, h, w, int(bool(flip)), float(fir_gain),
                                                _ptr(scale), _ptr(bias), _ptr(noise), nmode, float(noise_strength), a, al, g, cl,
                                                _ptr(residual), L.stream()), 'upfir_planar_sep')
diff --git a/sh-gan_amd/model_zoo/stylegan.py b/sh-gan_amd/model_zoo/stylegan.py
--- a/sh-gan_amd/model_zoo/stylegan.py
+++ b/sh-gan_amd/model_zoo/stylegan.py
@@ -204,7 +204,7 @@
             return kernels.conv2d(x, pw, mode=kernels.MODE_SAME, pad=padding, in_scale=s, out_scale=d, noise=noise,
                                   bias=ep.get('bias'), residual=ep.get('residual'),
                                   **{k: v for k, v in ep.items() if k in ('act', 'gain', 'alpha', 'act_gain', 'clamp')})
-        mid = kernels.conv2d(x, pw, mode=kernels.MODE_UP2T, in_scale=s, planar=True)
+        mid = kernels.conv2d(x, pw, mode=kernels.MODE_UP2T, in_scale=s, planar='pitch')
         return kernels.upfir_planar(mid, resample_filter, scale=d.reshape(-1) if d is not None else None, noise=noise,
                                     bias=ep.get('bias'), residual=ep.get('residual'),
                                     **{k: v for k, v in ep.items() if k in ('act', 'gain', 'alpha', 'act_gain', 'clamp')})
@@ -655,7 +655,7 @@
         if self.up == 1:
             return kernels.conv2d(x, pw, mode=kernels.MODE_SAME, pad=self.padding, in_scale=s, out_scale=d, noise=noise,
                                   noise_strength=ns, bias=b, residual=residual, **ak)
-        mid = kernels.conv2d(x, pw, mode=kernels.MODE_UP2T, in_scale=s, planar=True)
+        mid = kernels.conv2d(x, pw, mode=kernels.MODE_UP2T, in_scale=s, planar='pitch')
         return kernels.upfir_planar(mid, self.resample_filter, scale=d.reshape(-1), noise=noise, noise_strength=ns, bias=b,
                                     residual=residual, **ak)
 
```

After: 818.4 (median of 4 runs). No clear change (+0.3%).
